# octree-nn/octfusion

Measured on AMD Instinct MI355X. Metric: denoising-steps/sec (depth-8 octree, batch 8), higher is better.
Workload: dtype f32 storage, fp16x3 products (fp16 hi + lo operand pairs = 22 significand bits, three fp16 MFMAs per product, fp32 accumulate)

## Files before the change

include/ofx.h:

```cpp
#ifndef OFX_H_
#define OFX_H_

#include <stddef.h>
#include <stdint.h>

#ifdef __cplusplus
extern "C" {
#endif

#define OFX_OK 0
#define OFX_EINVAL (-1)
#define OFX_ELAUNCH (-2)
#define OFX_ENODEV (-3)

#define OFX_ACT_NONE 0
#define OFX_ACT_SILU 1
#define OFX_ACT_GELU 2

#define OFX_MAX_DEPTH 16

int ofx_version(void);
const char* ofx_status_string(int status);
int ofx_device_check(void);
const char* ofx_build_hash(void);
// ... 72 lines not shown
int ofx_graphconv_bwd_weight(const float* x, int64_t ldx, int cin, int64_t n_nodes, const int32_t* nbr,
                             const int32_t* seg_ptr, const int32_t* col, const int32_t* nbr_ext,
                             const int32_t* multi_seg, int64_t n_multi, float* aux, const float* type_frac, int64_t ldt,
                             int nt_pad, const float* dy, int64_t ldy, int cout, float* dWp, int64_t Kp, void* ws,
                             size_t ws_bytes, void* stream);
int ofx_gn_backward(const float* x, int64_t ldx, const float* dy, int64_t ldy, int64_t n, int C,
                    const int32_t* batch_id, int batch_size, const float* count, int groups, float count_eps,
                    const float* mean, const float* rstd, const float* w, const float* bias, int act, double* sums,
                    float* coef, float* dx, int64_t lddx, float* dgamma, float* dbeta, void* stream);
int ofx_gemm_tn_f32(const float* P, int64_t ldp, const float* Q, int64_t ldq, int64_t rows, int64_t K, int64_t N,
                    float* out, void* ws, size_t ws_bytes, void* stream);
int ofx_table_reverse_count(const int32_t* nbr, int64_t n_out, int ndir, int64_t n_in, int32_t* rev_cnt, void* stream);
int ofx_table_reverse_fill(const int32_t* nbr, int64_t n_out, int ndir, int64_t n_in, const int32_t* rev_ptr,
                           int32_t* cursor, int32_t* rev_row, float* rev_w, void* stream);
int ofx_seg_primary_w(const int32_t* seg_ptr, const int32_t* col, const float* w, int64_t nseg, int32_t* nbr,
                      void* stream);
int ofx_seg_multi_flag_w(const int32_t* seg_ptr, const float* w, int64_t nseg, int32_t* flag, void* stream);
int ofx_seg_primary_ext_w(const int32_t* seg_ptr, const int32_t* col, const float* w, int64_t nseg, int64_t n_src,
                          const int32_t* rank, int32_t* nbr_ext, int32_t* multi_seg, void* stream);
int ofx_gridconv_bwd_data(const float* dy, int64_t ldy, int cout, int64_t n_out, int64_t n_in, const int32_t* nbr_rev,
                          const int32_t* rev_ptr, const int32_t* rev_row, const float* rev_w,
                          const int32_t* nbr_ext_rev, const int32_t* multi_seg, int64_t n_multi, float* aux,
                          const float* WpT, int cin, float* dx, int64_t ldx, void* ws, size_t ws_bytes, void* stream);
int ofx_gridconv_bwd_weight(const float* x, int64_t ldx, int cin, int64_t n_in, int64_t n_out, const int32_t* nbr27,
                            const int32_t* nbr27_ext, const float* zero_row, const float* dy, int64_t ldy, int cout,
                            float* dWp, void* ws, size_t ws_bytes, void* stream);
int ofx_adamw_step(float* param, const float* grad, float* exp_avg, float* exp_avg_sq, int64_t n, float lr,
                   float beta1, float beta2, float eps, float weight_decay, int step, void* stream);
int ofx_ema_update(float* ema, const float* param, int64_t n, float beta, void* stream);
typedef struct OfxAdamRow {
  float* param;
  const float* grad;
  float* exp_avg;
  float* exp_avg_sq;
  float* ema;
  int64_t n;
} OfxAdamRow;
int ofx_adamw_ema_multi(const OfxAdamRow* rows, int64_t n_rows, float lr, float beta1, float beta2, float eps,
                        float weight_decay, int step, float ema_beta, void* stream);
int ofx_adamw_ema_multi_chunk(void);
int ofx_adamw_ema_multi_rows(void);
int64_t ofx_mse_grad_partials(int64_t n);
int ofx_mse_grad(const float* y, const float* target, float* dy, double* partials, double* loss_out, int64_t n,
                 void* stream);
int ofx_mpu_eval(const ofx_tree_t* tree, int depth_start, int depth_end, const float* pts, int64_t n_pts,
                 const float* code, float* sdf, uint8_t* mask, void* stream);
int ofx_mpu_eval_grid(const ofx_tree_t* tree, int depth_start, int depth_end, const float* code, int size,
                      float step, float bbmin, int batch_index, int64_t head, int64_t count, float* sdf,
                      uint8_t* mask, void* stream);
int ofx_mpu_eval_grad(const ofx_tree_t* tree, int depth_start, int depth_end, const float* pts, int64_t n_pts,
                      const float* code, float* sdf, float* grad, uint8_t* mask, void* stream);
int ofx_mpu_backward(const ofx_tree_t* tree, int depth_start, int depth_end, const float* pts, int64_t n_pts,
                     const float* code, const float* dsdf, const float* dgrad, float* dcode, void* stream);
int ofx_octree_ce(const float* logits, int64_t ld, const int32_t* child, int64_t n, float dscale, double* sums,
                  float* dlogits, int64_t ldd, void* stream);
int ofx_sdf_reg_loss(const float* sdf, const float* grad, const float* sdf_gt, const float* grad_gt, int64_t n,
                     float w_sdf, float w_grad, double* sums, float* dsdf, float* dgrad, void* stream);
int ofx_kl_sample_fwd(const float* params, int64_t ld, const float* noise, int64_t n, int embed_dim, float* z,
                      double* kl_sum, void* stream);
int ofx_kl_sample_bwd(const float* params, int64_t ld, const float* noise, const float* dz, int64_t n,
                      int embed_dim, float kl_scale, float* dparams, int64_t ldp, void* stream);
int ofx_graph_multi_flag(const int32_t* seg_ptr, int64_t n_nodes, int32_t* flag, void* stream);
int ofx_graph_primary_ext(const int32_t* seg_ptr, const int32_t* col, int64_t n_nodes,
                          const int32_t* rank, int32_t* nbr_ext, int32_t* multi_seg, void* stream);
int ofx_graph_type_frac(const int32_t* seg_ptr, const int32_t* col, const uint8_t* node_type,
                        int64_t n_nodes, int nt, float* type_frac, int64_t ld, void* stream);

int ofx_set_precision(int mode);
int ofx_get_precision(void);
int64_t ofx_packed_floats(int64_t Kp, int64_t N);
int64_t ofx_packed_k(int64_t K);
int64_t ofx_graphconv_packed_k(int cin, int nt);
int ofx_pack_weights(const float* W, int64_t sk, int64_t sn, int64_t K, int64_t N,
                     int cin, int nt, float* Wp, int64_t Kp, void* stream);

int ofx_gemm_f32(const float* A, int64_t lda, const int32_t* a_rows, int64_t M, int64_t K,
                 const float* Wp, int64_t Kp, int64_t N, const float* bias,
                 const float* res, int64_t ldr, float* out, int64_t ldc,
                 const int32_t* out_rows, void* ws, size_t ws_bytes, void* stream);
int ofx_gemm_f32_planes(const float* A, int64_t lda, const int32_t* a_rows, int64_t M, int64_t K,
                        const float* Wp, int64_t Kp, int64_t N, const float* bias,
                        const float* res, int64_t ldr, float* out, int64_t ldc,
                        const int32_t* out_rows, void* ws, size_t ws_bytes, int out_mode, void* stream);

int ofx_graphconv_fwd(const float* x, int64_t ldx, int cin, int64_t n_nodes,
                      const int32_t* nbr, const int32_t* seg_ptr, const int32_t* col,
                      const int32_t* nbr_ext, const int32_t* multi_seg, int64_t n_multi, float* aux,
                      const float* type_frac, int64_t ldt, int nt_pad,
                      const float* Wp, int64_t Kp, int cout, const float* bias,
                      const float* emb, int64_t lde, const int32_t* batch_id,
                      const float* res, int64_t ldr, float* out, int64_t ldc,
                      double* stats , int64_t stats_ld,
                      void* ws, size_t ws_bytes, void* stream);

int ofx_graphconv_narrow_in(const float* x, int64_t ldx, int cin, int64_t n_nodes, const int32_t* seg_ptr,
                            const int32_t* col, const uint8_t* node_type, int nt, const float* W, int cout,
                            const float* bias, const int32_t* batch_id, float* out, int64_t ldc,
                            double* stats , int64_t stats_ld, void* ws, size_t ws_bytes, void* stream);
int ofx_graphconv_narrow_in_tab(const float* x, int64_t ldx, int cin, int64_t n_nodes, const int32_t* seg_ptr,
                                const int32_t* col, const int32_t* nbr_ext, const int32_t* multi_seg, int64_t n_multi,
                                void* aux, const uint8_t* node_type, int nt, const float* W, int cout, const float* bias,
                                const int32_t* batch_id, float* out, int64_t ldc, double* stats ,
                                int64_t stats_ld, void* ws, size_t ws_bytes, void* stream);
int ofx_narrow_out_pack(const float* W, int C, int nt, int cout, int pw, float* Wd, void* stream);
int ofx_narrow_out_type_term(const float* type_frac, int64_t ldt, int nt, int64_t n_nodes, const float* W, int C,
                             int cout, const float* bias, float* type_term, void* stream);
int ofx_graphconv_narrow_out(const float* P, int64_t ldp, int cout, int64_t n_nodes, const int32_t* seg_ptr,
                             const int32_t* col, const float* type_term , float* out, int64_t ldc,
                             void* stream);

int ofx_planes_split(const float* x, int64_t ldx, int64_t n, int C, int Cpad, int mode, void* out,
                     int64_t ldo_bytes, void* stream);
int ofx_planes_merge(const void* planes, int64_t ldp_bytes, int64_t n, int C, int mode, float* out, int64_t ldo,
                     void* stream);
int ofx_gn_apply_planes(const float* x, int64_t ldx, int64_t n, int C, const int32_t* batch_id, const float* mean,
                        const float* rstd, const double* sums, const float* count, int groups, float eps,
                        float count_eps, const float* w, const float* bias, int act, int mode, void* out,
                        int64_t ldo_bytes, const int32_t* seg_ptr, const int32_t* col, const int32_t* multi_seg,
                        int64_t n_multi, void* aux , const int32_t* aux_plan ,
                        int64_t aux_left, void* stream);
int ofx_gn_apply_planes_oct(const float* x, int64_t ldx, int64_t n, int C, const int32_t* batch_id, const float* mean,
                            const float* rstd, const double* sums, const float* count, int groups, float eps,
                            float count_eps, const float* w, const float* bias, int act, int mode, void* out,
                            int64_t ldo_bytes, int64_t n_multi, void* aux, const int32_t* oct_ptr,
                            const int32_t* oct_ent, int64_t n_own, int shift, const int32_t* left_head,
                            const int32_t* left_src, int64_t n_left, void* stream);
int ofx_gn_finalize_window(const double* sums, const float* count, int batch_size, int C, int groups, int c_lo,
                           int c_hi, float eps, float count_eps, float* mean, float* rstd, void* stream);
int ofx_gn_apply_planes_window(const float* x, int64_t ldx, int64_t n, int C, int c_lo, int c_hi,
                               const int32_t* batch_id, const float* mean, const float* rstd, const double* sums,
                               const float* count, int groups, float eps, float count_eps, const float* w,
                               const float* bias, int act, int mode, void* out, int64_t ldo_bytes,
                               const int32_t* seg_ptr, const int32_t* col, const int32_t* multi_seg, int64_t n_multi,
                               void* aux, const int32_t* aux_plan, int64_t aux_left, void* stream);
int ofx_gn_apply_planes_oct_window(const float* x, int64_t ldx, int64_t n, int C, int c_lo, int c_hi,
                                   const int32_t* batch_id, const float* mean, const float* rstd, const double* sums,
                                   const float* count, int groups, float eps, float count_eps, const float* w,
                                   const float* bias, int act, int mode, void* out, int64_t ldo_bytes, int64_t n_multi,
                                   void* aux, const int32_t* oct_ptr, const int32_t* oct_ent, int64_t n_own, int shift,
                                   const int32_t* left_head, const int32_t* left_src, int64_t n_left, void* stream);
int ofx_gn_apply_rows(void);
int64_t ofx_planes_packed_ktiles(int cin, int nt, int mode);
int64_t ofx_planes_packed_bytes(int cin, int nt, int cout, int mode);
int ofx_pack_weights_planes(const float* W, int64_t sk, int64_t sn, int cin, int nt, int cout, int mode, void* out,
                            void* stream);
int ofx_graphconv_fwd_planes(const void* xp, int64_t ldx_bytes, int cin, int64_t n_nodes, const int32_t* seg_ptr,
                             const int32_t* col, const int32_t* nbr_ext, const int32_t* multi_seg, int64_t n_multi,
                             void* aux, size_t aux_bytes, const void* tfp, int64_t ldt_bytes, int nt, const void* W2,
                             int cout, const float* bias, const float* emb, int64_t lde, const int32_t* batch_id,
                             const float* res, int64_t ldr, float* out, int64_t ldc, double* stats ,
                             int64_t stats_ld, void* ws, size_t ws_bytes, void* sync , size_t sync_bytes,
                             int mode, int aux_ready, void* stream);
int ofx_graphconv_fwd_planes_cus(const void* xp, int64_t ldx_bytes, int cin, int64_t n_nodes, const int32_t* seg_ptr,
                                 const int32_t* col, const int32_t* nbr_ext, const int32_t* multi_seg, int64_t n_multi,
                                 void* aux, size_t aux_bytes, const void* tfp, int64_t ldt_bytes, int nt,
                                 const void* W2, int cout, const float* bias, const float* emb, int64_t lde,
                                 const int32_t* batch_id, const float* res, int64_t ldr, float* out, int64_t ldc,
                                 double* stats , int64_t stats_ld, void* ws, size_t ws_bytes,
                                 void* sync , size_t sync_bytes, int mode, int aux_ready, int cus,
                                 void* stream);
int ofx_set_gconv_persistent(int on);
int64_t ofx_gemm_planes_packed_bytes(int K, int N, int mode);
int ofx_pack_gemm_planes(const float* W, int64_t sk, int64_t sn, int K, int N, int mode, void* out, void* stream);
int ofx_gemm_planes(const void* ap, int64_t lda_bytes, int64_t n_a, int64_t M, int K, const int32_t* row_tab,
                    const void* W2, int N, const float* bias, float* out, int64_t ldc, int out_mode, void* ws,
                    size_t ws_bytes, void* sync, size_t sync_bytes, int mode, void* stream);
int ofx_set_gconv_cus(int cus);
int ofx_gconv3_plan(int64_t n_rows, int cout, int nkt, int wm, int ni, int cus, int32_t* out, int64_t out_len);
int ofx_set_gconv2_tile(int wm);

int ofx_grid_conv_table(int mode, int depth_out, int batch_size, int32_t pad, int32_t* nbr27,
                        void* stream);
int64_t ofx_conv3d_packed_k(int cin);
int ofx_pack_conv3d(const float* W, int cin, int cout, float* Wp, void* stream);
int ofx_gridconv_fwd(const float* x, int64_t ldx, int cin, int64_t n_in, int64_t n_out,
                     const int32_t* nbr27 ,
                     const int32_t* nbr27_ext ,
                     const float* zero_row ,
                     const float* Wp, int cout, const float* bias, const float* emb, int64_t lde,
                     const int32_t* batch_id, const float* res, int64_t ldr, float* out,
                     int64_t ldc, void* ws, size_t ws_bytes, void* stream);
int ofx_gather_gemm_f32(const float* x, int64_t ldx, int cin, int ntap, int64_t n_src, int64_t n_out, const int32_t* tab,
                        const float* zero_row, const float* Wp, int64_t Kp, int cout, const float* bias,
                        const float* res, int64_t ldr, float* out, int64_t ldc, const int32_t* out_rows, void* ws,
                        size_t ws_bytes, int out_mode, void* stream);
int ofx_set_attention_split(int on);
int ofx_attention(const float* qkv, int64_t ldq, int batch_size, int T, int heads, int ch,
                  float* out, int64_t ldo, void* stream);

int ofx_attention_bwd(const float* qkv, int64_t ldq, const float* dout, int64_t ldo, int batch_size, int T, int heads,
                      int ch, float* rowstat, float* dqkv, int64_t ldd, void* stream);

int ofx_gather_mean(const float* x, int64_t ldx, int cin, int64_t n_nodes,
                    const int32_t* seg_ptr, const int32_t* col, float* col_data,
                    void* stream);

int ofx_gn_stats(const float* x, int64_t ldx, int64_t n, int C, const int32_t* batch_id,
                 int batch_size, double* sums, void* stream);
int ofx_gn_stats_acc(const float* x, int64_t ldx, int64_t n, int C, const int32_t* batch_id, int batch_size,
                     double* sums, void* stream);
int ofx_gn_finalize(const double* sums, const float* count, int batch_size, int C, int groups,
                    float eps, float count_eps, float* mean, float* rstd, void* stream);
int ofx_gn_apply(const float* x, int64_t ldx, int64_t n, int C, const int32_t* batch_id,
                 const float* mean , const float* rstd , const double* sums ,
                 const float* count, int groups, float eps, float count_eps, const float* w, const float* bias,
                 int act, float* out, int64_t ldo, void* stream);

int ofx_gn_fused_rows(const float* x, int64_t ldx, int rows_per_batch, int batch_size, int C, int groups, float eps,
                      float count_eps, const float* w, const float* bias, int act, float* out, int64_t ldo,
                      void* stream);

int ofx_set_gn_rows16(int on);

int ofx_rows_copy(const float* src, int64_t lds, const int32_t* smap, float* dst, int64_t ldd,
                  const int32_t* dmap, int64_t n, int C, void* stream);
int ofx_rows_copy_planes(const float* src, int64_t lds, const int32_t* smap, float* dst, int64_t ldd,
                         const int32_t* dmap, int64_t n, int C, int mode, void* stream);
int ofx_act(const float* x, float* y, int64_t n, int act, void* stream);
int ofx_timestep_embedding(const float* t, int batch_size, int dim, float max_period,
                           float* out, void* stream);
int ofx_learned_sinusoid(const float* t, const float* w, int batch_size, int half, float* out, void* stream);
int ofx_linear_small(const float* a, int64_t lda, int M, int K, const float* W, int64_t ldw, int N, const float* bias,
                     const float* res, int64_t ldr, int act_in, int act_out, float* out, int64_t ldo, void* stream);
int ofx_ddim_eps_update(float* x, const float* eps, const float* coef, float* x0_out, int64_t n,
                        void* stream);
int ofx_ddim_x0_update(float* x, const float* x0, const float* noise, const float* coef,
                       int64_t n, void* stream);

size_t ofx_mc_ws_bytes(int batch, int size);
int ofx_mc_count(const float* sdf, int batch, int size, float level, void* ws, int64_t* counts, void* stream);
int ofx_mc_emit(const float* sdf, int batch, int size, float level, float step, float bbmin, float scale, void* ws,
                const int64_t* vert_off, const int64_t* tri_off, float* verts, int32_t* faces, void* stream);
int ofx_mc_table_host(int8_t* tri_table, uint8_t* ntri);

size_t ofx_mesh_cc_ws_bytes(int64_t total_verts, int64_t total_faces, int batch);
int ofx_mesh_cc_label(const int32_t* faces, const int64_t* vert_off, const int64_t* tri_off, int batch,
                      int64_t total_verts, int64_t total_faces, int32_t* label, void* ws, int32_t* status,
                      void* stream);
int ofx_mesh_cc_table(const int32_t* faces, const int32_t* label, const int64_t* vert_off, const int64_t* tri_off,
                      int batch, int64_t total_verts, int64_t total_faces, int32_t* comp_of_vert, int32_t* comp_off,
                      void* ws, const int32_t* status, void* stream);
int ofx_mesh_cc_stats(const float* verts, const int32_t* faces, const int32_t* label, const int64_t* vert_off,
                      const int64_t* tri_off, int batch, int64_t total_verts, int64_t total_faces, int64_t n_comp,
                      int32_t* table, void* ws, const int32_t* status, void* stream);
int ofx_mesh_cc_select(const float* verts, const int32_t* faces, const int32_t* label, const int64_t* vert_off,
                       const int64_t* tri_off, int batch, int64_t total_verts, int64_t total_faces,
                       int32_t* winner_label, int64_t* keep_counts, void* ws, const int32_t* status, void* stream);
int ofx_mesh_cc_extract(const float* verts, const int32_t* faces, const int64_t* vert_off, const int64_t* tri_off,
                        int batch, int64_t total_verts, int64_t total_faces, const int64_t* new_vert_off,
                        const int64_t* new_tri_off, float* out_verts, int32_t* out_faces, void* ws,
                        const int32_t* status, void* stream);

size_t ofx_voxmesh_ws_bytes(int batch, int depth, int weld);
int ofx_voxmesh_mask_keys(const int64_t* keys, int64_t n, int batch0, int batch, int depth, void* ws, void* stream);
int ofx_voxmesh_mask_dense(const float* occ, int batch, int depth, float threshold, void* ws, void* stream);
int ofx_voxmesh_count(int batch, int depth, int weld, void* ws, int64_t* counts, void* stream);
int ofx_voxmesh_emit(int batch, int depth, int weld, void* ws, const int64_t* vert_off, const int64_t* tri_off,
                     float* verts, int32_t* faces, void* stream);

#define OFX_EMD_MAX_POINTS 2048
size_t ofx_surface_sample_ws_bytes(int batch, int64_t total_faces);
int ofx_surface_sample(const float* verts, const int32_t* faces, const int64_t* offs, const int64_t* ids, int batch,
                       int64_t total_faces, int n, uint64_t seed, int normalize, void* ws, float* out, void* stream);
int ofx_surface_sample_oriented(const float* verts, const int32_t* faces, const int64_t* offs, const int64_t* ids,
                                int batch, int64_t total_faces, int n, uint64_t seed, int normalize, void* ws,
                                float* out, float* normals, void* stream);
int ofx_nn_matrix(const float* a, int64_t na, int n, const float* b, int64_t nb, int m, float* d, void* stream);
int ofx_emd_matrix(const float* x, int64_t nx, const float* y, int64_t ny, int n, int m, float* e, void* stream);
// ... 40 lines not shown
```

octfusion_amd/_lib.py:

```python
import ctypes
import os

import torch

_HERE = os.path.dirname(os.path.abspath(__file__))
LIB_PATH = os.environ.get('OFX_LIB', os.path.join(_HERE, 'libofx.so'))

c_p = ctypes.c_void_p
c_i = ctypes.c_int
c_l = ctypes.c_int64
c_f = ctypes.c_float
c_d = ctypes.c_double
c_sz = ctypes.c_size_t
c_u64 = ctypes.c_uint64


class OfxTree(ctypes.Structure):
    _fields_ = [('depth', c_i), ('full_depth', c_i), ('batch_size', c_i),
                ('child_all', c_p), ('key_all', c_p), ('leafrank_all', c_p),
                ('nnum_host', c_p), ('nnum_nempty_host', c_p)]


class OfxAdamRow(ctypes.Structure):
    _fields_ = [('param', c_p), ('grad', c_p), ('exp_avg', c_p), ('exp_avg_sq', c_p), ('ema', c_p), ('n', c_l)]
# ... 3 lines not shown
    'ofx_version': (c_i, [], False),
    'ofx_status_string': (ctypes.c_char_p, [c_i], False),
    'ofx_device_check': (c_i, [], False),
    'ofx_build_hash': (ctypes.c_char_p, [], False),
    'ofx_probe_mfma_sustained': (c_i, [c_i, c_i, c_p, c_p, c_p], True),
    'ofx_scan_ws_bytes': (c_sz, [c_l], False),
    'ofx_scan_i32': (c_i, [c_p, c_p, c_l, c_p, c_p], True),
    'ofx_octree_full_layer': (c_i, [c_i, c_i, c_p, c_p, c_p], True),
    'ofx_octree_split': (c_i, [c_p, c_l, c_p, c_p, c_p, c_p], True),
    'ofx_octree_grow': (c_i, [c_p, c_p, c_l, c_p, c_p, c_p], True),
    'ofx_split_small_label0': (c_i, [c_p, c_i, c_i, c_p, c_p], True),
    'ofx_split_small_label1': (c_i, [c_p, c_i, c_i, c_p, c_p, c_p], True),
    'ofx_split_large_label0': (c_i, [c_p, c_l, c_p, c_p], True),
    'ofx_split_large_label1': (c_i, [c_p, c_l, c_p, c_p, c_p], True),
    'ofx_octree2voxel_cf': (c_i, [c_p, c_l, c_i, c_i, c_i, c_p, c_p], True),
    'ofx_voxel2octree_cf': (c_i, [c_p, c_i, c_i, c_i, c_p, c_l, c_p], True),
    'ofx_points_sort_ws_bytes': (c_sz, [c_l], False),
    'ofx_points_keys': (c_i, [c_p, c_l, c_p, c_i, c_l, c_i, c_p, c_p, c_p], True),
    'ofx_points_sort': (c_i, [c_p, c_p, c_l, c_p, c_p, c_p, c_sz, c_p], True),
    'ofx_octree_label_from_points': (c_i, [c_p, c_l, c_p, c_l, c_i, c_i, c_p, c_p], True),
    'ofx_octree_point_features': (c_i, [c_p, c_p, c_l, c_p, c_l, c_p, c_l, c_p, c_l, c_i, c_p, c_p, c_p, c_p], True),
    'ofx_tree_leafrank_ws_bytes': (c_sz, [c_l], False),
    'ofx_tree_leafrank': (c_i, [c_p, c_p, c_i, c_p, c_p, c_p], True),
    'ofx_graph_nodes': (c_i, [ctypes.POINTER(OfxTree), c_i, c_p, c_p, c_p, c_p, c_p], True),
    'ofx_graph_count': (c_i, [ctypes.POINTER(OfxTree), c_i, c_p, c_p], True),
    'ofx_graph_reverse_count': (c_i, [c_p, c_p, c_l, c_p, c_p], True),
    'ofx_graph_reverse_fill': (c_i, [c_p, c_p, c_l, c_p, c_p, c_p, c_p, c_p], True),
    'ofx_graph_primary_w': (c_i, [c_p, c_p, c_p, c_l, c_p, c_p], True),
    'ofx_graph_multi_flag_w': (c_i, [c_p, c_p, c_l, c_p, c_p], True),
    'ofx_graph_primary_ext_w': (c_i, [c_p, c_p, c_p, c_l, c_p, c_p, c_p, c_p], True),
    'ofx_graphconv_bwd_data': (c_i, [c_p, c_l, c_i, c_l, c_p, c_p, c_p, c_p, c_p, c_p, c_l, c_p, c_p, c_l, c_i, c_p,
                                     c_l, c_p, c_sz, c_p], True),
    'ofx_graphconv_bwd_weight': (c_i, [c_p, c_l, c_i, c_l, c_p, c_p, c_p, c_p, c_p, c_l, c_p, c_p, c_l, c_i, c_p, c_l,
                                       c_i, c_p, c_l, c_p, c_sz, c_p], True),
    'ofx_gn_backward': (c_i, [c_p, c_l, c_p, c_l, c_l, c_i, c_p, c_i, c_p, c_i, c_f, c_p, c_p, c_p, c_p, c_i, c_p, c_p,
                              c_p, c_l, c_p, c_p, c_p], True),
    'ofx_gemm_tn_f32': (c_i, [c_p, c_l, c_p, c_l, c_l, c_l, c_l, c_p, c_p, c_sz, c_p], True),
    'ofx_table_reverse_count': (c_i, [c_p, c_l, c_i, c_l, c_p, c_p], True),
    'ofx_table_reverse_fill': (c_i, [c_p, c_l, c_i, c_l, c_p, c_p, c_p, c_p, c_p], True),
    'ofx_seg_primary_w': (c_i, [c_p, c_p, c_p, c_l, c_p, c_p], True),
    'ofx_seg_multi_flag_w': (c_i, [c_p, c_p, c_l, c_p, c_p], True),
    'ofx_seg_primary_ext_w': (c_i, [c_p, c_p, c_p, c_l, c_l, c_p, c_p, c_p, c_p], True),
    'ofx_gridconv_bwd_data': (c_i, [c_p, c_l, c_i, c_l, c_l, c_p, c_p, c_p, c_p, c_p, c_p, c_l, c_p, c_p, c_i, c_p, c_l,
                                    c_p, c_sz, c_p], True),
    'ofx_gridconv_bwd_weight': (c_i, [c_p, c_l, c_i, c_l, c_l, c_p, c_p, c_p, c_p, c_l, c_i, c_p, c_p, c_sz, c_p], True),
    'ofx_attention_bwd': (c_i, [c_p, c_l, c_p, c_l, c_i, c_i, c_i, c_i, c_p, c_p, c_l, c_p], True),
    'ofx_adamw_step': (c_i, [c_p, c_p, c_p, c_p, c_l, c_f, c_f, c_f, c_f, c_f, c_i, c_p], True),
    'ofx_ema_update': (c_i, [c_p, c_p, c_l, c_f, c_p], True),
    'ofx_adamw_ema_multi': (c_i, [c_p, c_l, c_f, c_f, c_f, c_f, c_f, c_i, c_f, c_p], True),
    'ofx_adamw_ema_multi_chunk': (c_i, [], False),
    'ofx_adamw_ema_multi_rows': (c_i, [], False),
    'ofx_mse_grad_partials': (c_l, [c_l], False),
    'ofx_mse_grad': (c_i, [c_p, c_p, c_p, c_p, c_p, c_l, c_p], True),
    'ofx_gn_fused_rows': (c_i, [c_p, c_l, c_i, c_i, c_i, c_i, c_f, c_f, c_p, c_p, c_i, c_p, c_l, c_p], True),
    'ofx_set_gn_rows16': (c_i, [c_i], True),
    'ofx_mpu_eval': (c_i, [ctypes.POINTER(OfxTree), c_i, c_i, c_p, c_l, c_p, c_p, c_p, c_p], True),
    'ofx_mpu_eval_grid': (c_i, [ctypes.POINTER(OfxTree), c_i, c_i, c_p, c_i, c_f, c_f, c_i, c_l, c_l, c_p, c_p, c_p], True),
    'ofx_mpu_eval_grad': (c_i, [ctypes.POINTER(OfxTree), c_i, c_i, c_p, c_l, c_p, c_p, c_p, c_p, c_p], True),
    'ofx_mpu_backward': (c_i, [ctypes.POINTER(OfxTree), c_i, c_i, c_p, c_l, c_p, c_p, c_p, c_p, c_p], True),
    'ofx_octree_ce': (c_i, [c_p, c_l, c_p, c_l, c_f, c_p, c_p, c_l, c_p], True),
    'ofx_sdf_reg_loss': (c_i, [c_p, c_p, c_p, c_p, c_l, c_f, c_f, c_p, c_p, c_p, c_p], True),
    'ofx_kl_sample_fwd': (c_i, [c_p, c_l, c_p, c_l, c_i, c_p, c_p, c_p], True),
    'ofx_kl_sample_bwd': (c_i, [c_p, c_l, c_p, c_p, c_l, c_i, c_f, c_p, c_l, c_p], True),
    'ofx_graph_fill': (c_i, [ctypes.POINTER(OfxTree), c_i, c_p, c_p, c_p], True),
    'ofx_graph_expand': (c_i, [c_p, c_l, c_p, c_p, c_p, c_p, c_p], True),
    'ofx_graph_type_frac': (c_i, [c_p, c_p, c_p, c_l, c_i, c_p, c_l, c_p], True),
    'ofx_set_precision': (c_i, [c_i], True),
    'ofx_set_range_words': (c_i, [c_p], True),
    'ofx_get_precision': (c_i, [], False),
    'ofx_gn_apply_rows': (c_i, [], False),
    'ofx_set_attention_split': (c_i, [c_i], True),
    'ofx_gather_gemm_f32': (c_i, [c_p, c_l, c_i, c_i, c_l, c_l, c_p, c_p, c_p, c_l, c_i, c_p, c_p, c_l, c_p, c_l, c_p, c_p, c_sz, c_i, c_p], True),
    'ofx_graphconv_narrow_in_tab': (c_i, [c_p, c_l, c_i, c_l, c_p, c_p, c_p, c_p, c_l, c_p, c_p, c_i, c_p, c_i, c_p, c_p, c_p, c_l, c_p, c_l,
                                          c_p, c_sz, c_p], True),
    'ofx_graphconv_narrow_in': (c_i, [c_p, c_l, c_i, c_l, c_p, c_p, c_p, c_i, c_p, c_i, c_p, c_p, c_p, c_l, c_p, c_l, c_p, c_sz, c_p], True),
    'ofx_narrow_out_pack': (c_i, [c_p, c_i, c_i, c_i, c_i, c_p, c_p], True),
    'ofx_narrow_out_type_term': (c_i, [c_p, c_l, c_i, c_l, c_p, c_i, c_i, c_p, c_p, c_p], True),
    'ofx_graphconv_narrow_out': (c_i, [c_p, c_l, c_i, c_l, c_p, c_p, c_p, c_p, c_l, c_p], True),
    'ofx_packed_floats': (c_l, [c_l, c_l], False),
    'ofx_packed_k': (c_l, [c_l], False),
    'ofx_graphconv_packed_k': (c_l, [c_i, c_i], False),
    'ofx_pack_weights': (c_i, [c_p, c_l, c_l, c_l, c_l, c_i, c_i, c_p, c_l, c_p], True),
    'ofx_gemm_f32': (c_i, [c_p, c_l, c_p, c_l, c_l, c_p, c_l, c_l, c_p, c_p, c_l, c_p, c_l, c_p, c_p, c_sz, c_p], True),
    'ofx_gemm_f32_planes': (c_i, [c_p, c_l, c_p, c_l, c_l, c_p, c_l, c_l, c_p, c_p, c_l, c_p, c_l, c_p, c_p, c_sz, c_i, c_p], True),
    'ofx_graphconv_fwd': (c_i, [c_p, c_l, c_i, c_l, c_p, c_p, c_p, c_p, c_p, c_l, c_p, c_p, c_l, c_i, c_p, c_l,
                                c_i, c_p, c_p, c_l, c_p, c_p, c_l, c_p, c_l, c_p, c_l, c_p, c_sz, c_p], True),
    'ofx_planes_split': (c_i, [c_p, c_l, c_l, c_i, c_i, c_i, c_p, c_l, c_p], True),
    'ofx_planes_merge': (c_i, [c_p, c_l, c_l, c_i, c_i, c_p, c_l, c_p], True),
    'ofx_gn_apply_planes': (c_i, [c_p, c_l, c_l, c_i, c_p, c_p, c_p, c_p, c_p, c_i, c_f, c_f, c_p, c_p, c_i, c_i, c_p,
                                  c_l, c_p, c_p, c_p, c_l, c_p, c_p, c_l, c_p], True),
    'ofx_gn_apply_planes_oct': (c_i, [c_p, c_l, c_l, c_i, c_p, c_p, c_p, c_p, c_p, c_i, c_f, c_f, c_p, c_p, c_i, c_i, c_p,
                                      c_l, c_l, c_p, c_p, c_p, c_l, c_i, c_p, c_p, c_l, c_p], True),
    'ofx_planes_packed_ktiles': (c_l, [c_i, c_i, c_i], False),
    'ofx_planes_packed_bytes': (c_l, [c_i, c_i, c_i, c_i], False),
    'ofx_pack_weights_planes': (c_i, [c_p, c_l, c_l, c_i, c_i, c_i, c_i, c_p, c_p], True),
    'ofx_graphconv_fwd_planes': (c_i, [c_p, c_l, c_i, c_l, c_p, c_p, c_p, c_p, c_l, c_p, c_sz, c_p, c_l, c_i, c_p, c_i,
                                       c_p, c_p, c_l, c_p, c_p, c_l, c_p, c_l, c_p, c_l, c_p, c_sz, c_p, c_sz, c_i, c_i,
                                       c_p], True),
    'ofx_graphconv_fwd_planes_cus': (c_i, [c_p, c_l, c_i, c_l, c_p, c_p, c_p, c_p, c_l, c_p, c_sz, c_p, c_l, c_i, c_p,
                                           c_i, c_p, c_p, c_l, c_p, c_p, c_l, c_p, c_l, c_p, c_l, c_p, c_sz, c_p, c_sz,
                                           c_i, c_i, c_i, c_p], True),
    'ofx_gn_finalize_window': (c_i, [c_p, c_p, c_i, c_i, c_i, c_i, c_i, c_f, c_f, c_p, c_p, c_p], True),
    'ofx_gn_apply_planes_window': (c_i, [c_p, c_l, c_l, c_i, c_i, c_i, c_p, c_p, c_p, c_p, c_p, c_i, c_f, c_f, c_p, c_p,
                                         c_i, c_i, c_p, c_l, c_p, c_p, c_p, c_l, c_p, c_p, c_l, c_p], True),
    'ofx_gn_apply_planes_oct_window': (c_i, [c_p, c_l, c_l, c_i, c_i, c_i, c_p, c_p, c_p, c_p, c_p, c_i, c_f, c_f, c_p,
                                             c_p, c_i, c_i, c_p, c_l, c_l, c_p, c_p, c_p, c_l, c_i, c_p, c_p, c_l, c_p],
                                       True),
    'ofx_set_gconv_persistent': (c_i, [c_i], True),
    'ofx_set_gconv_cus': (c_i, [c_i], True),
    'ofx_gemm_planes_packed_bytes': (c_l, [c_i, c_i, c_i], False),
    'ofx_pack_gemm_planes': (c_i, [c_p, c_l, c_l, c_i, c_i, c_i, c_p, c_p], True),
    'ofx_gemm_planes': (c_i, [c_p, c_l, c_l, c_l, c_i, c_p, c_p, c_i, c_p, c_p, c_l, c_i, c_p, c_sz, c_p, c_sz, c_i, c_p], False),
    'ofx_gconv3_plan': (c_i, [c_l, c_i, c_i, c_i, c_i, c_i, c_p, c_l], False),
    'ofx_set_gconv2_tile': (c_i, [c_i], True),
    'ofx_graph_multi_flag': (c_i, [c_p, c_l, c_p, c_p], True),
    'ofx_graph_primary_ext': (c_i, [c_p, c_p, c_l, c_p, c_p, c_p, c_p], True),
    'ofx_graph_primary': (c_i, [c_p, c_p, c_l, c_p, c_p], True),
    'ofx_grid_conv_table': (c_i, [c_i, c_i, c_i, c_i, c_p, c_p], True),
    'ofx_conv3d_packed_k': (c_l, [c_i], False),
    'ofx_pack_conv3d': (c_i, [c_p, c_i, c_i, c_p, c_p], True),
    'ofx_gridconv_fwd': (c_i, [c_p, c_l, c_i, c_l, c_l, c_p, c_p, c_p, c_p, c_i, c_p, c_p, c_l, c_p, c_p, c_l, c_p,
                               c_l, c_p, c_sz, c_p], True),
    'ofx_attention': (c_i, [c_p, c_l, c_i, c_i, c_i, c_i, c_p, c_l, c_p], True),
    'ofx_gather_mean': (c_i, [c_p, c_l, c_i, c_l, c_p, c_p, c_p, c_p], True),
    'ofx_gn_stats': (c_i, [c_p, c_l, c_l, c_i, c_p, c_i, c_p, c_p], True),
    'ofx_gn_stats_acc': (c_i, [c_p, c_l, c_l, c_i, c_p, c_i, c_p, c_p], True),
    'ofx_gn_finalize': (c_i, [c_p, c_p, c_i, c_i, c_i, c_f, c_f, c_p, c_p, c_p], True),
    'ofx_gn_apply': (c_i, [c_p, c_l, c_l, c_i, c_p, c_p, c_p, c_p, c_p, c_i, c_f, c_f, c_p, c_p, c_i, c_p, c_l, c_p], True),
    'ofx_rows_copy': (c_i, [c_p, c_l, c_p, c_p, c_l, c_p, c_l, c_i, c_p], True),
    'ofx_rows_copy_planes': (c_i, [c_p, c_l, c_p, c_p, c_l, c_p, c_l, c_i, c_i, c_p], True),
    'ofx_act': (c_i, [c_p, c_p, c_l, c_i, c_p], True),
    'ofx_timestep_embedding': (c_i, [c_p, c_i, c_i, c_f, c_p, c_p], True),
    'ofx_learned_sinusoid': (c_i, [c_p, c_p, c_i, c_i, c_p, c_p], True),
    'ofx_linear_small': (c_i, [c_p, c_l, c_i, c_i, c_p, c_l, c_i, c_p, c_p, c_l, c_i, c_i, c_p, c_l, c_p], True),
    'ofx_ddim_eps_update': (c_i, [c_p, c_p, c_p, c_p, c_l, c_p], True),
    'ofx_ddim_x0_update': (c_i, [c_p, c_p, c_p, c_p, c_l, c_p], True),
    'ofx_mc_ws_bytes': (c_sz, [c_i, c_i], False),
    'ofx_mc_count': (c_i, [c_p, c_i, c_i, c_f, c_p, c_p, c_p], True),
    'ofx_mc_emit': (c_i, [c_p, c_i, c_i, c_f, c_f, c_f, c_f, c_p, c_p, c_p, c_p, c_p, c_p], True),
    'ofx_mc_table_host': (c_i, [c_p, c_p], True),
    'ofx_mesh_cc_ws_bytes': (c_sz, [c_l, c_l, c_i], False),
    'ofx_mesh_cc_label': (c_i, [c_p, c_p, c_p, c_i, c_l, c_l, c_p, c_p, c_p, c_p], True),
    'ofx_mesh_cc_table': (c_i, [c_p, c_p, c_p, c_p, c_i, c_l, c_l, c_p, c_p, c_p, c_p, c_p], True),
    'ofx_mesh_cc_stats': (c_i, [c_p, c_p, c_p, c_p, c_p, c_i, c_l, c_l, c_l, c_p, c_p, c_p, c_p], True),
    'ofx_mesh_cc_select': (c_i, [c_p, c_p, c_p, c_p, c_p, c_i, c_l, c_l, c_p, c_p, c_p, c_p, c_p], True),
    'ofx_mesh_cc_extract': (c_i, [c_p, c_p, c_p, c_p, c_i, c_l, c_l, c_p, c_p, c_p, c_p, c_p, c_p, c_p], True),
    'ofx_voxmesh_ws_bytes': (c_sz, [c_i, c_i, c_i], False),
    'ofx_voxmesh_mask_keys': (c_i, [c_p, c_l, c_i, c_i, c_i, c_p, c_p], True),
    'ofx_voxmesh_mask_dense': (c_i, [c_p, c_i, c_i, c_f, c_p, c_p], True),
    'ofx_voxmesh_count': (c_i, [c_i, c_i, c_i, c_p, c_p, c_p], True),
    'ofx_voxmesh_emit': (c_i, [c_i, c_i, c_i, c_p, c_p, c_p, c_p, c_p, c_p], True),
    'ofx_surface_sample_ws_bytes':(c_sz, [c_i, c_l], False),
    'ofx_surface_sample': (c_i, [c_p, c_p, c_p, c_p, c_i, c_l, c_i, c_u64, c_i, c_p, c_p, c_p], True),
    'ofx_surface_sample_oriented': (c_i, [c_p, c_p, c_p, c_p, c_i, c_l, c_i, c_u64, c_i, c_p, c_p, c_p, c_p], True),
    'ofx_nn_matrix': (c_i, [c_p, c_l, c_i, c_p, c_l, c_i, c_p, c_p], True),
    'ofx_emd_matrix': (c_i, [c_p, c_l, c_p, c_l, c_i, c_i, c_p, c_p], True),
    'ofx_metrics_hash': (c_u64, [c_u64, c_l, c_l, c_i], False),
    'ofx_nn_search_qpass': (c_i, [], False),
    'ofx_nn_search_tile': (c_i, [], False),
    'ofx_nn_search_splits': (c_i, [c_i, c_l, c_l], False),
    'ofx_nn_search_ws_bytes': (c_sz, [c_l], False),
    'ofx_nn_search': (c_i, [c_p, c_p, c_p, c_p, c_i, c_l, c_l, c_l, c_i, c_p, c_p, c_p, c_p], True),
    'ofx_sdf_sample_ws_bytes': (c_sz, [c_l, c_i], False),
    'ofx_sdf_sample_nodes': (c_i, [c_p, c_i, c_p, c_l, c_p, c_i, c_i, c_i, c_u64, c_l, c_p, c_f, c_p, c_p, c_p, c_p, c_p,
                                   c_p], True),
    'ofx_sdf_sample_occu': (c_i, [c_p, c_i, c_l, c_u64, c_l, c_p, c_f, c_p, c_p, c_p], True),
# ... 106 lines not shown
```

octfusion_amd/csrc/ofx_gemm.hip:

```cpp
#include "ofx_gemm_common.h"

constexpr int BM = 128;
constexpr int BK = 32;
constexpr int A_LD = BK + 4;
constexpr int MODE_DENSE = 0;
constexpr int MODE_GATHER = 1;

struct TileCoords { int split, tm, tn; };
__device__ __forceinline__ TileCoords tile_coords(const GemmArgs& g) {
  const int ntile = g.ntm * g.ntn;
  int bid = ofx_xcd_swizzle(blockIdx.x, ntile * g.nsplit);
  const int split = bid / ntile;
  bid -= split * ntile;
  const int tm = bid / g.ntn;
  return {split, tm, bid - tm * g.ntn};
}

__device__ __forceinline__ void load_a_dense(const GemmArgs& g, int64_t m0, int64_t k0, float4 (&va)[4]) {
  const int c4 = threadIdx.x & 7, r0 = threadIdx.x >> 3;
  const int64_t k = k0 + c4 * 4;
  const bool vec = ((g.lda & 3) == 0) && (k + 3 < g.K) && ((((uintptr_t)g.A) & 15) == 0);
#pragma unroll
  for (int i = 0; i < 4; ++i) {
    const int64_t m = m0 + r0 + 32 * i;
    float4 v = f4zero();
    if (m < g.M) {
      const int64_t ar = g.a_rows ? (int64_t)g.a_rows[m] : m;
      const float* p = g.A + ar * g.lda + k;
      if (vec) {
        v = *reinterpret_cast<const float4*>(p);
      } else {
        if (k + 0 < g.K) v.x = p[0];
        if (k + 1 < g.K) v.y = p[1];
        if (k + 2 < g.K) v.z = p[2];
        if (k + 3 < g.K) v.w = p[3];
      }
    }
    va[i] = v;
  }
}

template <int BN>
__device__ __forceinline__ void load_b_tile(const GemmArgs& g, int64_t n0, int64_t k0, float4 (&vb)[BN / 32]) {
#pragma unroll
  for (int i = 0; i < BN / 32; ++i) {
    const int idx = threadIdx.x + 256 * i;
    const int kql = idx / BN, n = idx % BN;
    const int64_t nn = n0 + n;
    vb[i] = (nn < g.N) ? *reinterpret_cast<const float4*>(g.Wp + (((k0 >> 2) + kql) * g.N + nn) * 4) : f4zero();
  }
}

template <int WM, int WN, int MI, int NI>
__global__ void __launch_bounds__(256, 2) gemm_dense_generic_kernel(const GemmArgs g) {
  constexpr int BN = WN * NI * 32;
  static_assert(WM * MI * 32 == BM, "BM");
  extern __shared__ __attribute__((aligned(16))) float smem[];
  float* As = smem;
  float* Bs = smem + 2 * BM * A_LD;

  const TileCoords tc = tile_coords(g);
  const int split = tc.split;
  const int64_t m0 = (int64_t)tc.tm * BM, n0 = (int64_t)tc.tn * BN;

  const int lane = threadIdx.x & 63, wid = threadIdx.x >> 6;
  const int wm = wid / WN, wn = wid % WN;
  const int l31 = lane & 31, h = lane >> 5;
  const int c4 = threadIdx.x & 7, r0 = threadIdx.x >> 3;

  f32x16 acc[MI][NI];
#pragma unroll
  for (int i = 0; i < MI; ++i)
#pragma unroll
    for (int j = 0; j < NI; ++j)
#pragma unroll
      for (int r = 0; r < 16; ++r) acc[i][j][r] = 0.f;

  float4 va[4];
  float4 vb[BN / 32];
  const int nkt_all = (int)(g.Kp / BK);
  const int kt_begin = split * g.kt_per_split;
  const int kt_end = (kt_begin + g.kt_per_split < nkt_all) ? kt_begin + g.kt_per_split : nkt_all;

// ... 205 lines not shown
        va2 = ldg4(xp + src_off(ia2, ldx, n_src, aux_delta) + cc);
        va3 = ldg4(xp + src_off(ia3, ldx, n_src, aux_delta) + cc);
      }
      const int ktw0 = MODE == MODE_DENSE ? g_begin : d0 * tpd + g_begin / ndir;
      load_w(wp + (int64_t)ktw0 * 8 * Ncols * 4);
    }
    stage(a_st, b_st);
    ia0 = ib0; ia1 = ib1; ia2 = ib2; ia3 = ib3;
    __syncthreads();

    for (int kt = g_begin; kt < g_end; ++kt) {
      const int buf = (kt - g_begin) & 1;
      const int ktn = kt + 1 < nkt_g ? kt + 1 : nkt_g - 1;
      const int dn = ktn % ndir;
      const int d2 = (kt + 2 < nkt_g ? kt + 2 : nkt_g - 1) % ndir;
      if (MODE == MODE_DENSE) {
        int cc = ktn * BK + c4 * 4;
        cc = cc < kclamp ? cc : kclamp;
        va0 = ldg4(dp0 + cc); va1 = ldg4(dp1 + cc); va2 = ldg4(dp2 + cc); va3 = ldg4(dp3 + cc);
      } else {
        ib0 = t0[d2]; ib1 = t1[d2]; ib2 = t2[d2]; ib3 = t3[d2];
        const int cc = (ktn / ndir) * BK + c4 * 4;
        va0 = ldg4(xp + src_off(ia0, ldx, n_src, aux_delta) + cc);
        va1 = ldg4(xp + src_off(ia1, ldx, n_src, aux_delta) + cc);
        va2 = ldg4(xp + src_off(ia2, ldx, n_src, aux_delta) + cc);
        va3 = ldg4(xp + src_off(ia3, ldx, n_src, aux_delta) + cc);
      }
      const int ktw = MODE == MODE_DENSE ? ktn : dn * tpd + ktn / ndir;
      load_w(wp + (int64_t)ktw * 8 * Ncols * 4);
      __builtin_amdgcn_sched_barrier(0);
      mfma_tile<WM, WN, MI, NI>(a_ld + buf * BM * A_LD, b_ld + buf * 8 * BN * 4, acc);
      __builtin_amdgcn_sched_barrier(0);
      stage(a_st + (buf ^ 1) * BM * A_LD, b_st + (buf ^ 1) * 8 * BN * 4);
      ia0 = ib0; ia1 = ib1; ia2 = ib2; ia3 = ib3;
      __syncthreads();
    }
  }

  for (int kt = t_begin; kt < kt_end; ++kt) {
    const int cc = (kt - nkt_g) * BK + c4 * 4;
    va0 = ldg4(tfp + m_0 * ldt + cc);
    va1 = ldg4(tfp + m_1 * ldt + cc);
    va2 = ldg4(tfp + m_2 * ldt + cc);
    va3 = ldg4(tfp + m_3 * ldt + cc);
    load_w(wp + (int64_t)kt * 8 * Ncols * 4);
    stage(a_st, b_st);
    __syncthreads();
    mfma_tile<WM, WN, MI, NI>(a_ld, b_ld, acc);
    __syncthreads();
  }

  epilogue_store<WM, WN, MI, NI>(g, acc, m0, n0, wm, wn, l31, h, split);
}


typedef __bf16 bf16x8_t __attribute__((ext_vector_type(8)));
typedef _Float16 f16x8h_t __attribute__((ext_vector_type(8)));
typedef unsigned u32x4h __attribute__((ext_vector_type(4)));

template <int H16>
__device__ __forceinline__ void split16x4(const float4& v, uint2& hi, uint2& lo) {
  if constexpr (H16 == 0) {
    hi.x = g2_pk_bf16(v.x, v.y);
    hi.y = g2_pk_bf16(v.z, v.w);
    const float hx = g2_bf16_lo(hi.x), hy = g2_bf16_hi(hi.x);
    const float hz = g2_bf16_lo(hi.y), hw = g2_bf16_hi(hi.y);
    lo.x = g2_pk_bf16(v.x - hx, v.y - hy);
    lo.y = g2_pk_bf16(v.z - hz, v.w - hw);
  } else {
    hi.x = g2_pk_f16(v.x, v.y);
    hi.y = g2_pk_f16(v.z, v.w);
    lo.x = g2_pk_f16(v.x - g2_f16_lo(hi.x), v.y - g2_f16_hi(hi.x));
    lo.y = g2_pk_f16(v.z - g2_f16_lo(hi.y), v.w - g2_f16_hi(hi.y));
  }
}
template <int H16>
__device__ __forceinline__ f32x16 mfma16(u32x4h a, u32x4h b, f32x16 c) {
  if constexpr (H16 == 0)
    return __builtin_amdgcn_mfma_f32_32x32x16_bf16(__builtin_bit_cast(bf16x8_t, a), __builtin_bit_cast(bf16x8_t, b), c, 0, 0, 0);
  else
    return __builtin_amdgcn_mfma_f32_32x32x16_f16(__builtin_bit_cast(f16x8h_t, a), __builtin_bit_cast(f16x8h_t, b), c, 0, 0, 0);
}

template <int MODE, int WM, int WN, int MI, int NI, int H16>
__global__ void __launch_bounds__(256, 2) gemm_pairs_x3_kernel(const GemmArgs g) {
  constexpr int BN = WN * NI * 32;
  constexpr int A_BYTES = BM * 80;
  constexpr int BUF_BYTES = 2 * A_BYTES;
  static_assert(WM * MI * 32 == BM, "BM");
  extern __shared__ __attribute__((aligned(16))) char smem8[];
  typedef unsigned u32x4 __attribute__((ext_vector_type(4)));
  typedef const u32x4 __attribute__((address_space(1)))* gqp;

  const TileCoords tc = tile_coords(g);
  const int split = tc.split;
  const int64_t m0 = (int64_t)tc.tm * BM, n0 = (int64_t)tc.tn * BN;

  const int lane = threadIdx.x & 63, wid = threadIdx.x >> 6;
  const int wm = wid / WN, wn = wid % WN;
  const int l31 = lane & 31, h = lane >> 5;
  const int c4 = threadIdx.x & 7;
  const int r0 = ((threadIdx.x >> 4) & 3) + 8 * (threadIdx.x >> 6) + 4 * ((threadIdx.x >> 3) & 1);

  const gfp xp = (gfp)sgpr64((uint64_t)(MODE == MODE_DENSE ? g.A : g.x));
  const gfp tfp = (gfp)sgpr64((uint64_t)g.tf);
  const gqp w16 = (gqp)sgpr64((uint64_t)g.W16);
  const gip tab = (gip)sgpr64((uint64_t)g.nbr_ext);
  const int64_t ldx = (int64_t)sgpr64((uint64_t)(MODE == MODE_DENSE ? g.lda : g.ldx));
  const int64_t ldt = (int64_t)sgpr64((uint64_t)g.ldt), n_src = (int64_t)sgpr64((uint64_t)g.n_src);
  const int64_t Ncols = (int64_t)sgpr64((uint64_t)g.N);
  const int64_t lo_off = (int64_t)sgpr64((uint64_t)(g.Kp / 8 * g.N));
  const int64_t aux_delta = (int64_t)sgpr64((uint64_t)((g.aux - g.x) - g.n_src * g.ldx));
  const int ndir = g.ndir;

  f32x16 acc[MI][NI];
#pragma unroll
  for (int i = 0; i < MI; ++i)
#pragma unroll
    for (int j = 0; j < NI; ++j)
#pragma unroll
      for (int r = 0; r < 16; ++r) acc[i][j][r] = 0.f;

  const int nkt_all = (int)(g.Kp / BK);
  const int kt_begin = split * g.kt_per_split;
  const int kt_end = (kt_begin + g.kt_per_split < nkt_all) ? kt_begin + g.kt_per_split : nkt_all;
  const int tpd = MODE == MODE_DENSE ? nkt_all : g.cin / BK;
  const int nkt_g = MODE == MODE_DENSE ? nkt_all : ndir * tpd;
  const int g_begin = kt_begin < nkt_g ? kt_begin : nkt_g;
  const int g_end = kt_end < nkt_g ? kt_end : nkt_g;
  const int t_begin = kt_begin > nkt_g ? kt_begin : nkt_g;

  int64_t m_0 = m0 + r0, m_1 = m_0 + 32, m_2 = m_0 + 64, m_3 = m_0 + 96;
  const int64_t mmax = g.M - 1;
  m_0 = m_0 < mmax ? m_0 : mmax; m_1 = m_1 < mmax ? m_1 : mmax;
  m_2 = m_2 < mmax ? m_2 : mmax; m_3 = m_3 < mmax ? m_3 : mmax;
  const gip t0 = tab + m_0 * ndir;
  const gip t1 = tab + m_1 * ndir;
  const gip t2 = tab + m_2 * ndir;
  const gip t3 = tab + m_3 * ndir;
  int64_t dr0 = m_0, dr1 = m_1, dr2 = m_2, dr3 = m_3;
  if (MODE == MODE_DENSE && g.a_rows) { dr0 = g.a_rows[m_0]; dr1 = g.a_rows[m_1]; dr2 = g.a_rows[m_2]; dr3 = g.a_rows[m_3]; }
  const gfp dp0 = xp + dr0 * ldx, dp1 = xp + dr1 * ldx, dp2 = xp + dr2 * ldx, dp3 = xp + dr3 * ldx;
  const int kclamp = (int)g.K - 4;

  int64_t bcol[NI];
#pragma unroll
  for (int j = 0; j < NI; ++j) {
    int64_t nn = n0 + (wn * NI + j) * 32 + l31;
    bcol[j] = (nn < Ncols ? nn : Ncols - 1) + (int64_t)h * Ncols;
  }
  char* const a_st = smem8 + (r0 * 80 + c4 * 8);
  const char* const a_ld = smem8 + ((wm * MI * 32 + l31) * 80 + 16 * h);

  struct BFrag { u32x4 h[2][NI], l[2][NI]; };
  struct RegSet { float4 a0, a1, a2, a3; };
  struct IdxSet { uint32_t i0, i1, i2, i3; };

  auto load_bfrag = [&](int ktw, BFrag& F) {
    const gqp wk = w16 + (int64_t)ktw * 4 * Ncols;
#pragma unroll
    for (int c = 0; c < 2; ++c)
#pragma unroll
      for (int j = 0; j < NI; ++j) {
        F.h[c][j] = wk[(int64_t)(2 * c) * Ncols + bcol[j]];
        F.l[c][j] = wk[lo_off + (int64_t)(2 * c) * Ncols + bcol[j]];
      }
  };
  auto store_a = [&](int buf, const RegSet& R) {
    char* a = a_st + buf * BUF_BYTES;
    uint2 hi, lo;
    split16x4<H16>(R.a0, hi, lo);
    *reinterpret_cast<uint2*>(a) = hi; *reinterpret_cast<uint2*>(a + A_BYTES) = lo;
    split16x4<H16>(R.a1, hi, lo);
    *reinterpret_cast<uint2*>(a + 32 * 80) = hi; *reinterpret_cast<uint2*>(a + 32 * 80 + A_BYTES) = lo;
    split16x4<H16>(R.a2, hi, lo);
    *reinterpret_cast<uint2*>(a + 64 * 80) = hi; *reinterpret_cast<uint2*>(a + 64 * 80 + A_BYTES) = lo;
    split16x4<H16>(R.a3, hi, lo);
    *reinterpret_cast<uint2*>(a + 96 * 80) = hi; *reinterpret_cast<uint2*>(a + 96 * 80 + A_BYTES) = lo;
  };
  auto compute = [&](int buf, const BFrag& F) {
    const char* a = a_ld + buf * BUF_BYTES;
    u32x4h ah[2][MI], al[2][MI];
#pragma unroll
    for (int c = 0; c < 2; ++c)
#pragma unroll
      for (int i = 0; i < MI; ++i) {
        ah[c][i] = *reinterpret_cast<const u32x4h*>(a + i * 32 * 80 + 32 * c);
        al[c][i] = *reinterpret_cast<const u32x4h*>(a + i * 32 * 80 + 32 * c + A_BYTES);
      }
#pragma unroll
    for (int c = 0; c < 2; ++c) {
#pragma unroll
      for (int i = 0; i < MI; ++i)
#pragma unroll
        for (int j = 0; j < NI; ++j)
          acc[i][j] = mfma16<H16>(al[c][i], F.h[c][j], acc[i][j]);
#pragma unroll
      for (int i = 0; i < MI; ++i)
#pragma unroll
        for (int j = 0; j < NI; ++j)
          acc[i][j] = mfma16<H16>(ah[c][i], F.l[c][j], acc[i][j]);
#pragma unroll
      for (int i = 0; i < MI; ++i)
#pragma unroll
        for (int j = 0; j < NI; ++j)
          acc[i][j] = mfma16<H16>(ah[c][i], F.h[c][j], acc[i][j]);
    }
  };

  if (g_begin < g_end) {
    RegSet R0, R1;
    IdxSet I0 = {0, 0, 0, 0}, I1 = {0, 0, 0, 0};
    BFrag F0, F1;
    auto clampg = [&](int it) { return it < nkt_g ? it : nkt_g - 1; };
    auto ktw_of = [&](int it) {
      const int itc = clampg(it);
      return MODE == MODE_DENSE ? itc : (itc % ndir) * tpd + itc / ndir;
    };
    auto load_idx = [&](int it, IdxSet& I) {
      if (MODE == MODE_DENSE) return;
      const int dc = clampg(it) % ndir;
      I.i0 = (uint32_t)t0[dc]; I.i1 = (uint32_t)t1[dc]; I.i2 = (uint32_t)t2[dc]; I.i3 = (uint32_t)t3[dc];
    };
    auto load_rows = [&](int it, const IdxSet& I, RegSet& R) {
      const int itc = clampg(it);
      if (MODE == MODE_DENSE) {
        int cc = itc * BK + c4 * 4;
        cc = cc < kclamp ? cc : kclamp;
        R.a0 = ldg4(dp0 + cc); R.a1 = ldg4(dp1 + cc); R.a2 = ldg4(dp2 + cc); R.a3 = ldg4(dp3 + cc);
      } else {
        const int cc = (itc / ndir) * BK + c4 * 4;
        R.a0 = ldg4(xp + src_off(I.i0, ldx, n_src, aux_delta) + cc);
        R.a1 = ldg4(xp + src_off(I.i1, ldx, n_src, aux_delta) + cc);
        R.a2 = ldg4(xp + src_off(I.i2, ldx, n_src, aux_delta) + cc);
        R.a3 = ldg4(xp + src_off(I.i3, ldx, n_src, aux_delta) + cc);
      }
    };
    auto load_bchunk = [&](int ktw, int c, BFrag& F) {
      const gqp wk = w16 + (int64_t)ktw * 4 * Ncols + (int64_t)(2 * c) * Ncols;
#pragma unroll
      for (int j = 0; j < NI; ++j) { F.h[c][j] = wk[bcol[j]]; F.l[c][j] = wk[lo_off + bcol[j]]; }
    };
    auto store_half = [&](int buf, const float4& v0, const float4& v1, int row_off) {
      char* a = a_st + buf * BUF_BYTES + row_off * 80;
      uint2 hi, lo;
      split16x4<H16>(v0, hi, lo);
      *reinterpret_cast<uint2*>(a) = hi; *reinterpret_cast<uint2*>(a + A_BYTES) = lo;
      split16x4<H16>(v1, hi, lo);
      *reinterpret_cast<uint2*>(a + 32 * 80) = hi; *reinterpret_cast<uint2*>(a + 32 * 80 + A_BYTES) = lo;
    };
#define OFX_FENCE() __builtin_amdgcn_sched_barrier(0)
    auto step = [&](int it, int buf, const IdxSet& Iuse, IdxSet& Iload, const BFrag& Fcur, BFrag& Fnext,
                    RegSet& Rnew, const RegSet& Rold) {
      const char* a = a_ld + buf * BUF_BYTES;
      const int ktw = ktw_of(it + 1);
      u32x4h ah[2][MI], al[2][MI];
#pragma unroll
      for (int c = 0; c < 2; ++c)
#pragma unroll
        for (int i = 0; i < MI; ++i) {
          ah[c][i] = *reinterpret_cast<const u32x4h*>(a + i * 32 * 80 + 32 * c);
          al[c][i] = *reinterpret_cast<const u32x4h*>(a + i * 32 * 80 + 32 * c + A_BYTES);
        }
      load_idx(it + 3, Iload);
      OFX_FENCE();
#define OFX_MFMA_GROUP(AOP, BOP, C)                                                                        \
      _Pragma("unroll") for (int i = 0; i < MI; ++i)                                                        \
        _Pragma("unroll") for (int j = 0; j < NI; ++j)                                                      \
          acc[i][j] = mfma16<H16>(AOP[C][i], Fcur.BOP[C][j], acc[i][j]);
      OFX_MFMA_GROUP(al, h, 0);
      OFX_FENCE();
      load_bchunk(ktw, 0, Fnext);
      OFX_FENCE();
      OFX_MFMA_GROUP(ah, l, 0);
      OFX_FENCE();
      load_bchunk(ktw, 1, Fnext);
      OFX_FENCE();
      OFX_MFMA_GROUP(ah, h, 0);
      OFX_FENCE();
      load_rows(it + 2, Iuse, Rnew);
      OFX_FENCE();
      OFX_MFMA_GROUP(al, h, 1);
      OFX_FENCE();
      store_half(buf ^ 1, Rold.a0, Rold.a1, 0);
      OFX_FENCE();
      OFX_MFMA_GROUP(ah, l, 1);
      OFX_FENCE();
      store_half(buf ^ 1, Rold.a2, Rold.a3, 64);
      OFX_FENCE();
      OFX_MFMA_GROUP(ah, h, 1);
#undef OFX_MFMA_GROUP
      __syncthreads();
    };

    load_idx(g_begin, I0);
    load_idx(g_begin + 1, I1);
    OFX_FENCE();
    load_rows(g_begin, I0, R0);
    load_bchunk(ktw_of(g_begin), 0, F0);
    load_bchunk(ktw_of(g_begin), 1, F0);
    OFX_FENCE();
    load_idx(g_begin + 2, I0);
    OFX_FENCE();
    load_rows(g_begin + 1, I1, R1);
    OFX_FENCE();
    store_half(0, R0.a0, R0.a1, 0);
    store_half(0, R0.a2, R0.a3, 64);
    __syncthreads();
    int it = g_begin;
    for (; it + 1 < g_end; it += 2) {
      step(it, 0, I0, I1, F0, F1, R0, R1);
      step(it + 1, 1, I1, I0, F1, F0, R1, R0);
    }
    if (it < g_end) step(it, 0, I0, I1, F0, F1, R0, R1);
    __syncthreads();
#undef OFX_FENCE
  }

  for (int kt = t_begin; kt < kt_end; ++kt) {
    const int cc = (kt - nkt_g) * BK + c4 * 4;
    RegSet R;
    BFrag F;
    R.a0 = ldg4(tfp + m_0 * ldt + cc);
    R.a1 = ldg4(tfp + m_1 * ldt + cc);
    R.a2 = ldg4(tfp + m_2 * ldt + cc);
    R.a3 = ldg4(tfp + m_3 * ldt + cc);
    load_bfrag(kt, F);
    store_a(0, R);
    __syncthreads();
    compute(0, F);
    __syncthreads();
  }

  epilogue_store<WM, WN, MI, NI>(g, acc, m0, n0, wm, wn, l31, h, split);
}

__device__ __forceinline__ uint32_t bf16_rne_bits(float f) {
  const uint32_t u = __float_as_uint(f);
  return (u + 0x7fffu + ((u >> 16) & 1u)) >> 16;
}
__global__ void pack_bf16x3_kernel(const float* __restrict__ Wp, int64_t Kp, int64_t N, uint16_t* __restrict__ W16,
                                   int h16) {
  const int64_t total = Kp * N;
  const float wscale = h16 ? reinterpret_cast<const float*>(W16 + 2 * total)[1] : 1.f;
  for (int64_t t = (int64_t)blockIdx.x * blockDim.x + threadIdx.x; t < total; t += (int64_t)gridDim.x * blockDim.x) {
    const int64_t kg = t / (N * 8), rem = t - kg * N * 8;
    const int64_t n = rem / 8;
    const int kk = (int)(rem - n * 8);
    const int64_t k = kg * 8 + kk;
    const float w = Wp[((k >> 2) * N + n) * 4 + (k & 3)];
    if (h16) {
      const float ws = g2_sat16(w * wscale);
      const _Float16 hi = (_Float16)ws;
      const _Float16 lo = (_Float16)(ws - (float)hi);
      W16[t] = __builtin_bit_cast(unsigned short, hi);
      W16[total + t] = __builtin_bit_cast(unsigned short, lo);
    } else {
      const uint32_t hi = bf16_rne_bits(w);
      const float wl = w - __uint_as_float(hi << 16);
      W16[t] = (uint16_t)hi;
      W16[total + t] = (uint16_t)bf16_rne_bits(wl);
    }
  }
}
static int g_precision = 3;
static int pack_bf16x3(const float* Wp, int64_t Kp, int64_t N, hipStream_t st) {
  uint16_t* W16 = reinterpret_cast<uint16_t*>(const_cast<float*>(Wp) + Kp * N);
  if (ofx_launch_weight_scale(Wp, 1, 0, Kp * N, 1, g_precision == 3 ? 1 : 0, const_cast<float*>(Wp) + 2 * Kp * N, st))
    return OFX_ELAUNCH;
  pack_bf16x3_kernel<<<ofx_grid(Kp * N, 256), 256, 0, st>>>(Wp, Kp, N, W16, g_precision == 3 ? 1 : 0);
  return hipGetLastError() == hipSuccess ? OFX_OK : OFX_ELAUNCH;
}

extern "C" int ofx_set_precision(int mode) {
  if (mode < 0 || mode > 3) return OFX_EINVAL;
  g_precision = mode;
  return OFX_OK;
}
extern "C" int ofx_get_precision(void) { return g_precision; }
extern "C" int64_t ofx_packed_floats(int64_t Kp, int64_t N) { return 2 * Kp * N + 32; }

__global__ void __launch_bounds__(256) multi_mean_kernel(const float* __restrict__ x, int64_t ldx, int cin,
                                                         const int32_t* __restrict__ seg_ptr,
                                                         const int32_t* __restrict__ col,
                                                         const int32_t* __restrict__ multi_seg, int64_t V,
                                                         float* __restrict__ aux, int64_t ldaux,
                                                         const float* __restrict__ w) {
  const int c4n = cin >> 2;
  const int64_t total = (V + 1) * c4n;
  for (int64_t t = (int64_t)blockIdx.x * blockDim.x + threadIdx.x; t < total; t += (int64_t)gridDim.x * blockDim.x) {
    const int64_t v = t / c4n;
    const int c = (int)(t - v * c4n) * 4;
    float4 acc = f4zero();
    if (v > 0) {
      const int64_t s = multi_seg[v - 1];
      const int32_t a = seg_ptr[s], e = seg_ptr[s + 1];
      if (w) {
        for (int32_t p = a; p < e; ++p) {
          const float wp = w[p];
          const float4 xv = *reinterpret_cast<const float4*>(x + (int64_t)col[p] * ldx + c);
          acc.x += wp * xv.x; acc.y += wp * xv.y; acc.z += wp * xv.z; acc.w += wp * xv.w;
        }
      } else {
        for (int32_t p = a; p < e; ++p) f4add(acc, *reinterpret_cast<const float4*>(x + (int64_t)col[p] * ldx + c));
        const float inv = 1.f / (float)(e - a);
        acc.x *= inv; acc.y *= inv; acc.z *= inv; acc.w *= inv;
      }
    }
    *reinterpret_cast<float4*>(aux + v * ldaux + c) = acc;
  }
}

__global__ void __launch_bounds__(256) splitk_reduce_kernel(const GemmArgs g) {
  const int64_t total = g.M * g.N;
  for (int64_t t = (int64_t)blockIdx.x * blockDim.x + threadIdx.x; t < total; t += (int64_t)gridDim.x * blockDim.x) {
    const int64_t m = t / g.N, n = t - m * g.N;
    float v = 0.f;
    for (int s = 0; s < g.nsplit; ++s) v += g.ws[(int64_t)s * total + t];
    if (g.oscale_p) v *= *g.oscale_p;
    if (g.bias) v += g.bias[n];
    if (g.emb) v += g.emb[(int64_t)g.bid[m] * g.lde + n];
    if (g.res) v += g.res[m * g.ldr + n];
    int64_t om = m;
    if (g.out_rows) { om = g.out_rows[m]; if (om < 0) continue; }
    g.out[om * g.ldc + n] = v;
  }
}

__global__ void __launch_bounds__(256) splitk_reduce_v4_kernel(const GemmArgs g) {
  const int64_t n4 = g.N >> 2, total4 = g.M * n4, total = g.M * g.N;
  for (int64_t t = (int64_t)blockIdx.x * blockDim.x + threadIdx.x; t < total4; t += (int64_t)gridDim.x * blockDim.x) {
    const int64_t m = t / n4, n = (t - m * n4) * 4;
    const float* p = g.ws + m * g.N + n;
    float4 v = f4zero();
    int s = 0;
    for (; s + 7 < g.nsplit; s += 8) {
      float4 a[8];
#pragma unroll
      for (int u = 0; u < 8; ++u) a[u] = *reinterpret_cast<const float4*>(p + (int64_t)(s + u) * total);
#pragma unroll
      for (int u = 0; u < 8; ++u) f4add(v, a[u]);
    }
    for (; s + 3 < g.nsplit; s += 4) {
      const float4 a0 = *reinterpret_cast<const float4*>(p + (int64_t)s * total);
      const float4 a1 = *reinterpret_cast<const float4*>(p + (int64_t)(s + 1) * total);
      const float4 a2 = *reinterpret_cast<const float4*>(p + (int64_t)(s + 2) * total);
      const float4 a3 = *reinterpret_cast<const float4*>(p + (int64_t)(s + 3) * total);
      f4add(v, a0); f4add(v, a1); f4add(v, a2); f4add(v, a3);
    }
    for (; s < g.nsplit; ++s) f4add(v, *reinterpret_cast<const float4*>(p + (int64_t)s * total));
    if (g.oscale_p) { const float osc = *g.oscale_p; v.x *= osc; v.y *= osc; v.z *= osc; v.w *= osc; }
    if (g.bias) f4add(v, *reinterpret_cast<const float4*>(g.bias + n));
    if (g.emb) f4add(v, *reinterpret_cast<const float4*>(g.emb + (int64_t)g.bid[m] * g.lde + n));
    if (g.res) f4add(v, *reinterpret_cast<const float4*>(g.res + m * g.ldr + n));
    int64_t om = m;
    if (g.out_rows) { om = g.out_rows[m]; if (om < 0) continue; }
    if (g.out_planes) ofx_store_planes4(g.out, om * g.ldc + n, v, g.out_planes);
    else *reinterpret_cast<float4*>(g.out + om * g.ldc + n) = v;
  }
}

template <void (*KERNEL)(const GemmArgs), size_t LDS>
static int launch_tiled(GemmArgs& g, hipStream_t st) {
  static bool attr_set[OFX_MAX_DEVICES] = {};
  if (LDS > 64 * 1024 &&
      !ofx_raise_lds_limit(reinterpret_cast<const void*>(KERNEL), (int)LDS, attr_set))
    return OFX_ELAUNCH;
  KERNEL<<<g.ntm * g.ntn * g.nsplit, 256, LDS, st>>>(g);
  return OFX_OK;
}
template <int MODE, int WM, int WN, int MI, int NI>
static int launch_cfg(GemmArgs& g, int flavour, hipStream_t st) {
  constexpr size_t lds_f32 = (2 * BM * A_LD + 2 * 8 * (WN * NI * 32) * 4) * sizeof(float);
  constexpr size_t lds_16 = 2 * (2 * BM * 80);
  switch (flavour) {
    case 3: return launch_tiled<gemm_pairs_x3_kernel<MODE, WM, WN, MI, NI, 1>, lds_16>(g, st);
    case 2: return launch_tiled<gemm_pairs_x3_kernel<MODE, WM, WN, MI, NI, 0>, lds_16>(g, st);
    case 1: return launch_tiled<gemm_fast_kernel<MODE, WM, WN, MI, NI>, lds_f32>(g, st);
  }
  if constexpr (MODE == MODE_DENSE) return launch_tiled<gemm_dense_generic_kernel<WM, WN, MI, NI>, lds_f32>(g, st);
  return OFX_EINVAL;
}

__global__ void __launch_bounds__(256) stats_reduce_kernel(const float* __restrict__ part, int64_t nwr, int wr_rows,
                                                            int64_t N, const int32_t* __restrict__ bid,
                                                            double* __restrict__ stats, int64_t stats_ld) {
  __shared__ double red[3][64][2];
  const int c = threadIdx.x & 63, rg = threadIdx.x >> 6;
  const int64_t n = (int64_t)blockIdx.y * 64 + c;
  const int64_t w0 = (int64_t)blockIdx.x * 64;
  const int64_t nc = n < N ? n : N - 1;
  int b[16];
  float2 v[16];
#pragma unroll
  for (int i = 0; i < 16; ++i) {
    const int64_t w = w0 + rg * 16 + i;
    const int64_t wc = w < nwr ? w : nwr - 1;
    b[i] = bid[wc * wr_rows];
    v[i] = *reinterpret_cast<const float2*>(part + (wc * N + nc) * 2);
    if (w >= nwr) { b[i] = -1; v[i] = make_float2(0.f, 0.f); }
  }
  const int bfirst = bid[w0 * wr_rows];
  bool ok = true;
#pragma unroll
  for (int i = 0; i < 16; ++i) ok = ok && (b[i] == bfirst || b[i] < 0);
  const bool uni = __syncthreads_and(ok);
  auto flush = [&](int bb, double s, double q) {
    double* o = stats + ((int64_t)bb * stats_ld + n) * 2;
    unsafeAtomicAdd(o, s); unsafeAtomicAdd(o + 1, q);
  };
  if (uni) {
    double s = 0.0, q = 0.0;
#pragma unroll
    for (int i = 0; i < 16; ++i) { s += (double)v[i].x; q += (double)v[i].y; }
    if (rg > 0) { red[rg - 1][c][0] = s; red[rg - 1][c][1] = q; }
    __syncthreads();
    if (rg == 0 && n < N) {
#pragma unroll
      for (int r = 0; r < 3; ++r) { s += red[r][c][0]; q += red[r][c][1]; }
      flush(bfirst, s, q);
    }
  } else if (n < N) {
    double s = 0.0, q = 0.0;
    int sb = -1;
#pragma unroll
    for (int i = 0; i < 16; ++i) {
      if (b[i] < 0) continue;
      if (b[i] != sb) {
        if (sb >= 0) flush(sb, s, q);
        sb = b[i]; s = 0.0; q = 0.0;
      }
      s += (double)v[i].x; q += (double)v[i].y;
    }
    if (sb >= 0) flush(sb, s, q);
  }
}

int ofx_launch_stats_reduce(const GemmArgs& g, int wr_rows, hipStream_t st) {
  const int64_t nwr = ofx_cdiv(g.M, wr_rows);
  stats_reduce_kernel<<<dim3((unsigned)ofx_cdiv(nwr, 64), (unsigned)ofx_cdiv(g.N, 64)), 256, 0, st>>>(
      g.stats_part, nwr, wr_rows, g.N, g.bid, g.stats, g.stats_ld);
  OFX_LAUNCH_CHECK();
  return OFX_OK;
}

template <int MODE>
static int launch_gemm(GemmArgs& g, float* ws, size_t ws_bytes, hipStream_t st) {
  if (g.M <= 0 || g.N <= 0) return OFX_OK;
  if (MODE == MODE_GATHER && !(g.fast && g.nbr_ext && g.aux && (!g.out_rows || g.gather_out_rows))) return OFX_EINVAL;
  {
    auto al16 = [](const void* p) { return (reinterpret_cast<uintptr_t>(p) & 15) == 0; };
    g.vec4 = g.N % 4 == 0 && al16(g.out) && g.ldc % 4 == 0 && (!g.res || (al16(g.res) && g.ldr % 4 == 0)) &&
             (!g.emb || (al16(g.emb) && g.lde % 4 == 0)) && (!g.bias || al16(g.bias));
  }
  const int bn = g.N <= 32 ? 32 : (g.N <= 64 ? 64 : 128);
  g.ntm = (int)ofx_cdiv(g.M, BM);
  g.ntn = (int)ofx_cdiv(g.N, bn);
  const int nkt = (int)(g.Kp / BK);
  int nsplit = 1;
  const int tiles = g.ntm * g.ntn;
  if (ws && tiles < 256 && nkt >= 8) {
    nsplit = (int)ofx_cdiv(512, tiles);
    if (nsplit > nkt / 4) nsplit = nkt / 4;
    if (nsplit > 64) nsplit = 64;
    const size_t per = (size_t)g.M * g.N * sizeof(float);
    if ((size_t)nsplit * per > ws_bytes) nsplit = (int)(ws_bytes / per);
    if (nsplit < 2) nsplit = 1;
  }
  g.kt_per_split = (int)ofx_cdiv(nkt, nsplit);
  nsplit = (int)ofx_cdiv(nkt, g.kt_per_split);
  g.nsplit = nsplit;
  g.ws = ws;
  bool fast = true;
  if (MODE == MODE_DENSE) {
    fast = ((g.lda & 3) == 0) && ((g.K & 3) == 0) && g.K >= 4 && ((((uintptr_t)g.A) & 15) == 0);
    if (fast) { g.ndir = 1; g.n_src = 0; g.aux = g.A; g.tf = g.A; g.ldt = g.lda; g.nbr_ext = (const int32_t*)g.A; }
  }
  g.W16 = (g_precision != 1) ? reinterpret_cast<const uint16_t*>(g.Wp + g.Kp * g.N) : nullptr;
  const int wr_rows = bn == 32 ? 32 : 64;
  const int64_t nwr = ofx_cdiv(g.M, wr_rows);
  if (!(g.stats && g.vec4 && nsplit == 1 && g.stats_part &&
        (size_t)nwr * g.N * 2 * sizeof(float) <= g.stats_part_bytes && (((uintptr_t)g.stats_part) & 15) == 0))
    g.stats_part = nullptr;
  g.oscale_p = (fast && g.W16) ? g.Wp + 2 * g.Kp * g.N : nullptr;
  const int flavour = !fast ? 0 : (!g.W16 ? 1 : (g_precision == 3 ? 3 : 2));
  int rc;
  if (bn == 32) rc = launch_cfg<MODE, 4, 1, 1, 1>(g, flavour, st);
  else if (bn == 64) rc = launch_cfg<MODE, 2, 2, 2, 1>(g, flavour, st);
  else rc = launch_cfg<MODE, 2, 2, 2, 2>(g, flavour, st);
  if (rc) return rc;
  if (nsplit > 1) {
    const bool ws16 = (((uintptr_t)g.ws) & 15) == 0;
    if (g.vec4 && ws16) splitk_reduce_v4_kernel<<<ofx_grid(g.M * (g.N >> 2), 256), 256, 0, st>>>(g);
    else splitk_reduce_kernel<<<ofx_grid(g.M * g.N, 256), 256, 0, st>>>(g);
  }
  if (g.stats_part) {
    rc = ofx_launch_stats_reduce(g, wr_rows, st);
    if (rc) return rc;
  }
  OFX_LAUNCH_CHECK();
  return OFX_OK;
}

static inline int64_t pad32(int64_t v) { return (v + 31) / 32 * 32; }

extern "C" int64_t ofx_packed_k(int64_t K) { return pad32(K); }
extern "C" int64_t ofx_graphconv_packed_k(int cin, int nt) {
  return pad32(7 * (int64_t)cin) + (nt > 1 ? pad32(7 * (int64_t)nt) : 0);
}

__global__ void pack_weights_kernel(const float* __restrict__ W, int64_t sk, int64_t sn, int64_t K, int64_t N, int cin,
                                    int nt, float* __restrict__ Wp, int64_t Kp) {
  const int64_t total = (Kp / 4) * N;
  const int ntc = nt > 1 ? nt : 0;
  const int64_t Kf = (7 * (int64_t)cin + 31) / 32 * 32;
  for (int64_t t = (int64_t)blockIdx.x * blockDim.x + threadIdx.x; t < total; t += (int64_t)gridDim.x * blockDim.x) {
    const int64_t kq = t / N, n = t - kq * N;
    float v[4];
#pragma unroll
    for (int kk = 0; kk < 4; ++kk) {
      const int64_t k = kq * 4 + kk;
      int64_t src = -1;
      if (cin > 0) {
        if (k < 7 * (int64_t)cin) {
          const int64_t dir = k / cin, c = k - dir * cin;
          src = dir * (cin + ntc) + c;
        } else if (k >= Kf && ntc > 0 && k - Kf < 7 * (int64_t)ntc) {
          const int64_t kt = k - Kf, dir = kt / ntc, ty = kt - dir * ntc;
          src = dir * (cin + ntc) + cin + ty;
        }
      } else if (k < K) {
        src = k;
      }
      v[kk] = src >= 0 ? W[src * sk + n * sn] : 0.f;
    }
    *reinterpret_cast<float4*>(Wp + t * 4) = make_float4(v[0], v[1], v[2], v[3]);
  }
}

extern "C" int ofx_pack_weights(const float* W, int64_t sk, int64_t sn, int64_t K, int64_t N, int cin, int nt,
                                float* Wp, int64_t Kp, void* stream) {
  if (!W || !Wp || K < 1 || N < 1 || (Kp & 31) || cin < 0 || nt < 0) return OFX_EINVAL;
  if (cin > 0) {
    if (Kp != ofx_graphconv_packed_k(cin, nt) || K != 7 * (int64_t)(cin + (nt > 1 ? nt : 0))) return OFX_EINVAL;
  } else if (Kp != pad32(K)) {
    return OFX_EINVAL;
  }
  if (((uintptr_t)Wp & 15) != 0) return OFX_EINVAL;
  pack_weights_kernel<<<ofx_grid((Kp / 4) * N, 256), 256, 0, ofx_stream(stream)>>>(W, sk, sn, K, N, cin, nt, Wp, Kp);
  if (int rc = pack_bf16x3(Wp, Kp, N, ofx_stream(stream))) return rc;
  OFX_LAUNCH_CHECK();
  return OFX_OK;
}

__global__ void pack_conv3d_kernel(const float* __restrict__ W, int cin, int64_t N, float* __restrict__ Wp, int64_t Kp) {
  const int64_t total = (Kp / 4) * N;
  for (int64_t t = (int64_t)blockIdx.x * blockDim.x + threadIdx.x; t < total; t += (int64_t)gridDim.x * blockDim.x) {
    const int64_t kq = t / N, n = t - kq * N;
    float v[4];
#pragma unroll
    for (int kk = 0; kk < 4; ++kk) {
      const int64_t k = kq * 4 + kk;
      float w = 0.f;
      if (k < 27 * (int64_t)cin) {
        const int64_t tap = k / cin, c = k - tap * cin;
        w = W[(n * cin + c) * 27 + tap];
      }
      v[kk] = w;
    }
    *reinterpret_cast<float4*>(Wp + t * 4) = make_float4(v[0], v[1], v[2], v[3]);
  }
}

extern "C" int64_t ofx_conv3d_packed_k(int cin) { return pad32(27 * (int64_t)cin); }

extern "C" int ofx_pack_conv3d(const float* W, int cin, int cout, float* Wp, void* stream) {
  if (!W || !Wp || cin < 1 || cout < 1 || ((uintptr_t)Wp & 15)) return OFX_EINVAL;
  const int64_t Kp = ofx_conv3d_packed_k(cin);
  pack_conv3d_kernel<<<ofx_grid((Kp / 4) * cout, 256), 256, 0, ofx_stream(stream)>>>(W, cin, cout, Wp, Kp);
  if (int rc = pack_bf16x3(Wp, Kp, cout, ofx_stream(stream))) return rc;
  OFX_LAUNCH_CHECK();
  return OFX_OK;
}

extern "C" int ofx_gemm_f32_planes(const float* A, int64_t lda, const int32_t* a_rows, int64_t M, int64_t K,
                                   const float* Wp, int64_t Kp, int64_t N, const float* bias, const float* res, int64_t ldr,
                                   float* out, int64_t ldc, const int32_t* out_rows, void* ws, size_t ws_bytes,
                                   int out_mode, void* stream) {
  if (M == 0 && K >= 1 && N >= 1) return OFX_OK;
  if (M < 0 || K < 1 || N < 1 || !Wp || !out || (M > 0 && !A) || Kp != pad32(K) || lda < K || ldc < N ||
      (res && ldr < N) || ((uintptr_t)Wp & 15))
    return OFX_EINVAL;
  if (out_mode != 0 && out_mode != 2 && out_mode != 3) return OFX_EINVAL;
  if (out_mode && ((N & 3) || (ldc & 31) || ((uintptr_t)out & 127) || (res && ((ldr & 3) || ((uintptr_t)res & 15))) ||
                   (bias && ((uintptr_t)bias & 15)) || ((uintptr_t)ws & 15)))
    return OFX_EINVAL;
  GemmArgs g = {};
  g.A = A; g.lda = lda; g.a_rows = a_rows;
  g.M = M; g.K = K; g.Wp = Wp; g.Kp = Kp; g.N = N; g.bias = bias;
  g.res = res; g.ldr = ldr; g.out = out; g.ldc = ldc; g.out_rows = out_rows; g.out_planes = out_mode;
  return launch_gemm<MODE_DENSE>(g, (float*)ws, ws_bytes, ofx_stream(stream));
}
extern "C" int ofx_gemm_f32(const float* A, int64_t lda, const int32_t* a_rows, int64_t M, int64_t K, const float* Wp,
                            int64_t Kp, int64_t N, const float* bias, const float* res, int64_t ldr, float* out,
                            int64_t ldc, const int32_t* out_rows, void* ws, size_t ws_bytes, void* stream) {
  return ofx_gemm_f32_planes(A, lda, a_rows, M, K, Wp, Kp, N, bias, res, ldr, out, ldc, out_rows, ws, ws_bytes, 0, stream);
}

static int gather_common(GemmArgs& g, const float* x, int64_t ldx, int cin, int ndir, int64_t n_rows,
                         const int32_t* nbr, const int32_t* seg_ptr, const int32_t* col, const float* Wp, int64_t Kp,
                         int cout, const float* bias, const float* emb, int64_t lde, const int32_t* batch_id,
                         const float* res, int64_t ldr, float* out, int64_t ldc) {
  if (n_rows < 0 || cin < 1 || cout < 1 || !x || !nbr || !Wp || !out || ldx < cin || ldc < cout ||
      (res && ldr < cout) || (emb && (!batch_id || lde < cout)) || ((uintptr_t)Wp & 15))
    return OFX_EINVAL;
  g.x = x; g.ldx = ldx; g.cin = cin; g.ndir = ndir;
  g.fast = (cin % 32 == 0) && ((ldx & 3) == 0) && (((uintptr_t)x & 15) == 0);
  g.nbr = nbr; g.seg_ptr = seg_ptr; g.col = col;
  g.Kf = pad32((int64_t)ndir * cin);
  g.M = n_rows; g.K = Kp; g.Wp = Wp; g.Kp = Kp; g.N = cout; g.bias = bias;
  g.emb = emb; g.lde = lde; g.bid = batch_id; g.res = res; g.ldr = ldr; g.out = out; g.ldc = ldc;
  return OFX_OK;
}

__device__ __forceinline__ float gather_elem(const GemmArgs& g, int64_t row, int64_t k) {
  if (k >= (int64_t)g.ndir * g.cin) return 0.f;
  const int dir = (int)(k / g.cin), c = (int)(k - (int64_t)dir * g.cin);
  const int32_t nb = g.nbr[row * g.ndir + dir];
  if (nb >= 0) return g.x[(int64_t)nb * g.ldx + c];
  if (nb == -1) return 0.f;
  const int64_t s = row * g.ndir + dir;
  const int32_t a = g.seg_ptr[s], e = g.seg_ptr[s + 1];
  float acc = 0.f;
  if (g.edge_w) {
    for (int32_t p = a; p < e; ++p) acc += g.edge_w[p] * g.x[(int64_t)g.col[p] * g.ldx + c];
    return acc;
  }
  for (int32_t p = a; p < e; ++p) acc += g.x[(int64_t)g.col[p] * g.ldx + c];
  if (e - a > 1) acc /= (float)(e - a);
  return acc;
}
__global__ void __launch_bounds__(256) col_rows_kernel(const GemmArgs g, int64_t row0, int64_t rows,
                                                       float* __restrict__ colbuf) {
  const int64_t k4n = g.Kp >> 2, total = rows * k4n;
  for (int64_t t = (int64_t)blockIdx.x * blockDim.x + threadIdx.x; t < total; t += (int64_t)gridDim.x * blockDim.x) {
    const int64_t r = t / k4n, k = (t - r * k4n) * 4;
    const int64_t row = row0 + r;
    float v[4];
#pragma unroll
    for (int kk = 0; kk < 4; ++kk)
      v[kk] = (k + kk < g.Kf) ? gather_elem(g, row, k + kk) : g.tf[row * g.ldt + (k + kk - g.Kf)];
    *reinterpret_cast<float4*>(colbuf + t * 4) = make_float4(v[0], v[1], v[2], v[3]);
  }
}

static int launch_gather_via_col(const GemmArgs& g, float* ws, size_t ws_bytes, hipStream_t st) {
  if (!ws || (((uintptr_t)ws) & 15)) return OFX_EINVAL;
  size_t tail = ws_bytes / 8;
  if (tail > (size_t(16) << 20)) tail = size_t(16) << 20;
  tail &= ~size_t(15);
  const size_t row_bytes = (size_t)g.Kp * sizeof(float);
  int64_t chunk = (int64_t)((ws_bytes - tail) / row_bytes) / 128 * 128;
  if (chunk < 128) return OFX_EINVAL;
  float* tail_ws = reinterpret_cast<float*>(reinterpret_cast<char*>(ws) + (ws_bytes - tail));
  for (int64_t r0 = 0; r0 < g.M; r0 += chunk) {
    const int64_t rows = g.M - r0 < chunk ? g.M - r0 : chunk;
    col_rows_kernel<<<ofx_grid(rows * (g.Kp >> 2), 256), 256, 0, st>>>(g, r0, rows, ws);
    GemmArgs d = {};
    d.A = ws; d.lda = g.Kp; d.M = rows; d.K = g.Kp; d.Wp = g.Wp; d.Kp = g.Kp; d.N = g.N; d.bias = g.bias;
    d.emb = g.emb; d.lde = g.lde; d.bid = g.bid ? g.bid + r0 : nullptr;
    d.res = g.res ? g.res + r0 * g.ldr : nullptr; d.ldr = g.ldr;
    d.out = g.out + r0 * g.ldc; d.ldc = g.ldc;
    d.stats = g.stats; d.stats_ld = g.stats_ld;
    if (g.stats) { d.stats_part = tail_ws; d.stats_part_bytes = tail; }
    const int rc = launch_gemm<MODE_DENSE>(d, g.stats ? nullptr : tail_ws, tail, st);
    if (rc) return rc;
  }
  return OFX_OK;
}

extern "C" int ofx_graphconv_fwd(const float* x, int64_t ldx, int cin, int64_t n_nodes, const int32_t* nbr,
                                 const int32_t* seg_ptr, const int32_t* col, const int32_t* nbr_ext,
                                 const int32_t* multi_seg, int64_t n_multi, float* aux, const float* type_frac,
                                 int64_t ldt, int nt_pad, const float* Wp, int64_t Kp, int cout, const float* bias,
// ... 358 lines not shown
    a.rows_per_slice = ofx_cdiv(ofx_cdiv(rows, slices), 32) * 32;
    const int sl = (int)ofx_cdiv(rows, a.rows_per_slice);
    launch_tn<true>(a, dim3((unsigned)ofx_cdiv(Kp, 128), (unsigned)ofx_cdiv(cout, 128), (unsigned)sl), st);
    tn_reduce_kernel<<<ofx_grid(total, 256), 256, 0, st>>>(a.part, sl, total, dWp, first ? 0 : 1);
    first = 0;
  }
  OFX_LAUNCH_CHECK();
  return OFX_OK;
}

extern "C" int ofx_gemm_tn_f32(const float* P, int64_t ldp, const float* Q, int64_t ldq, int64_t rows, int64_t K,
                               int64_t N, float* out, void* ws, size_t ws_bytes, void* stream) {
  if (rows < 0 || K < 4 || N < 4 || (K & 3) || (N & 3) || !out || !ws || ldp < K || ldq < N || ((ldp | ldq) & 3) ||
      (rows > 0 && (!P || !Q)) || (((uintptr_t)P | (uintptr_t)Q | (uintptr_t)ws) & 15))
    return OFX_EINVAL;
  hipStream_t st = ofx_stream(stream);
  const int64_t total = K * N;
  if (rows == 0) {
    if (hipMemsetAsync(out, 0, (size_t)total * sizeof(float), st) != hipSuccess) return OFX_ELAUNCH;
    return OFX_OK;
  }
  const int tiles = (int)(ofx_cdiv(K, 128) * ofx_cdiv(N, 128));
  int slices = (int)ofx_cdiv(1024, tiles);
  if (slices > 256) slices = 256;
  if (slices > (int)ofx_cdiv(rows, 32)) slices = (int)ofx_cdiv(rows, 32);
  while (slices > 1 && (size_t)slices * total * sizeof(float) > ws_bytes) --slices;
  if ((size_t)slices * total * sizeof(float) > ws_bytes) return OFX_EINVAL;
  TnArgs a = {};
  a.P = P; a.ldp = ldp; a.Q = Q; a.ldq = ldq; a.Kp = K; a.N = N; a.Kf = K; a.rows = rows; a.row0 = 0;
  a.rows_per_slice = ofx_cdiv(ofx_cdiv(rows, slices), 32) * 32;
  slices = (int)ofx_cdiv(rows, a.rows_per_slice);
  a.part = (float*)ws;
  launch_tn<true>(a, dim3((unsigned)ofx_cdiv(K, 128), (unsigned)ofx_cdiv(N, 128), (unsigned)slices), st);
  tn_reduce_kernel<<<ofx_grid(total, 256), 256, 0, st>>>(a.part, slices, total, out, 0);
  OFX_LAUNCH_CHECK();
  return OFX_OK;
}

extern "C" int ofx_gridconv_fwd(const float* x, int64_t ldx, int cin, int64_t n_in, int64_t n_out,
                                const int32_t* nbr27, const int32_t* nbr27_ext, const float* zero_row,
                                const float* Wp, int cout,
                                const float* bias, const float* emb, int64_t lde, const int32_t* batch_id,
                                const float* res, int64_t ldr, float* out, int64_t ldc, void* ws, size_t ws_bytes,
                                void* stream) {
  if (n_out == 0 && cin >= 1 && cout >= 1) return OFX_OK;
  GemmArgs g = {};
  const int64_t Kp = ofx_conv3d_packed_k(cin);
  int rc = gather_common(g, x, ldx, cin, 27, n_out, nbr27 ? nbr27 : nbr27_ext, nullptr, nullptr, Wp, Kp, cout, bias,
                         emb, lde, batch_id, res, ldr, out, ldc);
  if (rc) return rc;
  if (n_in < 1) return OFX_EINVAL;
  if (g.fast && nbr27_ext && zero_row && (((uintptr_t)zero_row & 15) == 0)) {
    g.nbr_ext = nbr27_ext; g.aux = zero_row; g.ldaux = ldx; g.n_src = n_in;
    g.tf = x; g.ldt = ldx;
    return launch_gemm<MODE_GATHER>(g, (float*)ws, ws_bytes, ofx_stream(stream));
  }
  if (!nbr27) return OFX_EINVAL;
  return launch_gather_via_col(g, (float*)ws, ws_bytes, ofx_stream(stream));
}

extern "C" int ofx_gather_gemm_f32(const float* x, int64_t ldx, int cin, int ntap, int64_t n_src, int64_t n_out,
                                   const int32_t* tab, const float* zero_row, const float* Wp, int64_t Kp, int cout,
                                   const float* bias, const float* res, int64_t ldr, float* out, int64_t ldc,
                                   const int32_t* out_rows, void* ws, size_t ws_bytes, int out_mode, void* stream) {
  if (n_out == 0 && cin >= 1 && cout >= 1) return OFX_OK;
  if (ntap < 1 || ntap > 64 || n_src < 1 || !tab || !zero_row || ((uintptr_t)zero_row & 15) || (cin & 31) || (ldx & 3) ||
      ((uintptr_t)x & 15) || Kp != pad32((int64_t)ntap * cin))
    return OFX_EINVAL;
  if (out_mode != 0 && out_mode != 2 && out_mode != 3) return OFX_EINVAL;
  if (out_mode && ((cout & 3) || (ldc & 31) || ((uintptr_t)out & 127) || (res && ((ldr & 3) || ((uintptr_t)res & 15))) ||
                   (bias && ((uintptr_t)bias & 15)) || ((uintptr_t)ws & 15)))
    return OFX_EINVAL;
  GemmArgs g = {};
  int rc = gather_common(g, x, ldx, cin, ntap, n_out, tab, nullptr, nullptr, Wp, Kp, cout, bias, nullptr, 0, nullptr, res,
                         ldr, out, ldc);
  if (rc) return rc;
  if (!g.fast) return OFX_EINVAL;
  g.nbr_ext = tab; g.aux = zero_row; g.ldaux = ldx; g.n_src = n_src;
  g.tf = x; g.ldt = ldx;
  g.out_rows = out_rows; g.gather_out_rows = 1; g.out_planes = out_mode;
  return launch_gemm<MODE_GATHER>(g, (float*)ws, ws_bytes, ofx_stream(stream));
}

__global__ void __launch_bounds__(256) gather_mean_kernel(const float* __restrict__ x, int64_t ldx, int cin, int64_t nseg,
                                                          const int32_t* __restrict__ seg_ptr,
                                                          const int32_t* __restrict__ col, float* __restrict__ out) {
  const int c4n = cin >> 2;
  const int64_t total = nseg * c4n;
  for (int64_t t = (int64_t)blockIdx.x * blockDim.x + threadIdx.x; t < total; t += (int64_t)gridDim.x * blockDim.x) {
    const int64_t s = t / c4n;
    const int c = (int)(t - s * c4n) * 4;
    const int32_t a = seg_ptr[s], e = seg_ptr[s + 1];
    float4 acc = f4zero();
    for (int32_t p = a; p < e; ++p) f4add(acc, *reinterpret_cast<const float4*>(x + (int64_t)col[p] * ldx + c));
    if (e - a > 1) {
      const float inv = 1.f / (float)(e - a);
      acc.x *= inv; acc.y *= inv; acc.z *= inv; acc.w *= inv;
    }
    *reinterpret_cast<float4*>(out + s * cin + c) = acc;
  }
}
__global__ void __launch_bounds__(256) gather_mean_scalar_kernel(const float* __restrict__ x, int64_t ldx, int cin,
                                                                 int64_t nseg, const int32_t* __restrict__ seg_ptr,
                                                                 const int32_t* __restrict__ col,
                                                                 float* __restrict__ out) {
  const int64_t total = nseg * cin;
  for (int64_t t = (int64_t)blockIdx.x * blockDim.x + threadIdx.x; t < total; t += (int64_t)gridDim.x * blockDim.x) {
    const int64_t s = t / cin;
    const int c = (int)(t - s * cin);
    const int32_t a = seg_ptr[s], e = seg_ptr[s + 1];
    float acc = 0.f;
    for (int32_t p = a; p < e; ++p) acc += x[(int64_t)col[p] * ldx + c];
    if (e - a > 1) acc /= (float)(e - a);
    out[t] = acc;
  }
}

extern "C" int ofx_gather_mean(const float* x, int64_t ldx, int cin, int64_t n_nodes, const int32_t* seg_ptr,
                               const int32_t* col, float* col_data, void* stream) {
  if (!x || !seg_ptr || !col || !col_data || cin < 1 || ldx < cin || n_nodes < 0) return OFX_EINVAL;
  const int64_t nseg = n_nodes * 7;
  hipStream_t st = ofx_stream(stream);
  const bool vec = (cin % 4 == 0) && ((ldx & 3) == 0) && (((uintptr_t)x & 15) == 0) && (((uintptr_t)col_data & 15) == 0);
  if (vec)
    gather_mean_kernel<<<ofx_grid(nseg * (cin / 4), 256), 256, 0, st>>>(x, ldx, cin, nseg, seg_ptr, col, col_data);
  else
    gather_mean_scalar_kernel<<<ofx_grid(nseg * cin, 256), 256, 0, st>>>(x, ldx, cin, nseg, seg_ptr, col, col_data);
  OFX_LAUNCH_CHECK();
  return OFX_OK;
}
```

octfusion_amd/csrc/ofx_gemm_common.h:

```cpp
#pragma once
#include "ofx_common.h"

typedef float f32x16 __attribute__((ext_vector_type(16)));

struct GemmArgs {
  const float* A; int64_t lda; const int32_t* a_rows;
  const float* x; int64_t ldx; int cin; int ndir; int fast;
  const int32_t* nbr;
  const int32_t* seg_ptr; const int32_t* col;
  const float* edge_w;
  const float* tf; int64_t ldt; int64_t Kf;
  const int32_t* nbr_ext;
  const float* aux; int64_t ldaux; int64_t n_src;
  int64_t M, K;
  const float* Wp; int64_t Kp, N;
  const uint16_t* W16;
  const float* oscale_p;
  const float* bias;
  const float* emb; int64_t lde; const int32_t* bid;
  const float* res; int64_t ldr;
  float* out; int64_t ldc; const int32_t* out_rows;
  int gather_out_rows;
  int out_planes;
  double* stats; int64_t stats_ld;
  int ntm, ntn, nsplit, kt_per_split;
  float* ws;
  int vec4;
  float* stats_part; size_t stats_part_bytes;
};

static __global__ void __launch_bounds__(256) weight_absmax_kernel(const float* __restrict__ W, int64_t sk, int64_t sn, int64_t K,
                                                            int64_t N, unsigned* __restrict__ acc) {
  __shared__ float red[256];
  float m = 0.f;
  for (int64_t t = (int64_t)blockIdx.x * 256 + threadIdx.x; t < K * N; t += (int64_t)gridDim.x * 256) {
    const float a = fabsf(W[(t / N) * sk + (t % N) * sn]);
    if (a <= 3.0e38f) m = fmaxf(m, a);
  }
  red[threadIdx.x] = m;
  __syncthreads();
  for (int o = 128; o > 0; o >>= 1) {
    if ((int)threadIdx.x < o) red[threadIdx.x] = fmaxf(red[threadIdx.x], red[threadIdx.x + o]);
    __syncthreads();
  }
  if (threadIdx.x == 0) atomicMax(acc, __float_as_uint(red[0]));
}
static __global__ void weight_scale_finish_kernel(int fp16_operands, float* __restrict__ scale) {
  const float mx = __uint_as_float(reinterpret_cast<const unsigned*>(scale)[0]);
  float s = 1.f;
  if (fp16_operands && mx > 0.f) {
    int e;
    frexpf(mx, &e);
    int sh = 15 - e;
    sh = sh < -60 ? -60 : (sh > 60 ? 60 : sh);
    s = ldexpf(1.f, sh);
  }
  scale[0] = 1.f / s;
  scale[1] = s;
}
static inline int ofx_launch_weight_scale(const float* W, int64_t sk, int64_t sn, int64_t K, int64_t N, int fp16_operands,
                                          float* scale, hipStream_t st) {
  if (hipMemsetAsync(scale, 0, sizeof(float), st) != hipSuccess) return OFX_ELAUNCH;
  int64_t nb = (K * N + 256 * 16 - 1) / (256 * 16);
  nb = nb < 1 ? 1 : (nb > 1024 ? 1024 : nb);
  weight_absmax_kernel<<<(unsigned)nb, 256, 0, st>>>(W, sk, sn, K, N, reinterpret_cast<unsigned*>(scale));
  if (hipGetLastError() != hipSuccess) return OFX_ELAUNCH;
  weight_scale_finish_kernel<<<1, 1, 0, st>>>(fp16_operands, scale);
  if (hipGetLastError() != hipSuccess) return OFX_ELAUNCH;
  return OFX_OK;
}


__device__ __forceinline__ unsigned g2_pk_bf16(float a, float b) {
  unsigned r;
  asm("v_cvt_pk_bf16_f32 %0, %1, %2" : "=v"(r) : "v"(a), "v"(b));
  return r;
}
__device__ __forceinline__ unsigned g2_pk_f16(float a, float b) {
  const _Float16 x = (_Float16)a, y = (_Float16)b;
  return (unsigned)__builtin_bit_cast(unsigned short, x) | ((unsigned)__builtin_bit_cast(unsigned short, y) << 16);
}
__device__ __forceinline__ float g2_bf16_lo(unsigned p) { return __uint_as_float(p << 16); }
__device__ __forceinline__ float g2_bf16_hi(unsigned p) { return __uint_as_float(p & 0xffff0000u); }
__device__ __forceinline__ float g2_f16_lo(unsigned p) { return (float)__builtin_bit_cast(_Float16, (unsigned short)(p & 0xffffu)); }
__device__ __forceinline__ float g2_f16_hi(unsigned p) { return (float)__builtin_bit_cast(_Float16, (unsigned short)(p >> 16)); }
__device__ __forceinline__ float g2_sat16(float v) { return fminf(fmaxf(v, -65504.f), 65504.f); }
__device__ __forceinline__ void g2_split2(int mode, float a, float b, unsigned& hi, unsigned& lo) {
  if (mode == 3) {
    hi = g2_pk_f16(a, b);
    lo = g2_pk_f16(a - g2_f16_lo(hi), b - g2_f16_hi(hi));
  } else {
    hi = g2_pk_bf16(a, b);
    lo = g2_pk_bf16(a - g2_bf16_lo(hi), b - g2_bf16_hi(hi));
  }
}
__device__ __forceinline__ void g2_join2(int mode, unsigned hi, unsigned lo, float& a, float& b) {
  if (mode == 3) { a = g2_f16_lo(hi) + g2_f16_lo(lo); b = g2_f16_hi(hi) + g2_f16_hi(lo); }
  else { a = g2_bf16_lo(hi) + g2_bf16_lo(lo); b = g2_bf16_hi(hi) + g2_bf16_hi(lo); }
}
__host__ __device__ static inline bool g2_pairs(int mode) { return mode == 2 || mode == 3; }

__device__ __forceinline__ void ofx_store_planes4(float* base, int64_t f, const float4& v, int mode) {
  unsigned h0, h1, l0, l1;
  g2_split2(mode, v.x, v.y, h0, l0);
  g2_split2(mode, v.z, v.w, h1, l1);
  char* o = reinterpret_cast<char*>(base) + (f >> 5) * 128 + (f & 31) * 2;
  *reinterpret_cast<uint2*>(o) = make_uint2(h0, h1);
  *reinterpret_cast<uint2*>(o + 64) = make_uint2(l0, l1);
}

__device__ __forceinline__ int ofx_xcd_swizzle(int bid, int n) {
  const int q = n / 8, r = n % 8, xcd = bid % 8, j = bid / 8;
  return (xcd < r ? xcd * (q + 1) : r * (q + 1) + (xcd - r) * q) + j;
// ... 183 lines not shown
```

octfusion_amd/csrc/ofx_norm.hip:

```cpp
#include "ofx_planes.h"

constexpr int GN_ROWS_PER_BLOCK = 64;

static inline int64_t gn_stats_rows(int64_t n, int batch_size, int C = 128) {
  const int64_t chunks = (n + GN_ROWS_PER_BLOCK - 1) / GN_ROWS_PER_BLOCK;
  const int64_t bytes_per_batch = n * (int64_t)C * 4 / (batch_size > 0 ? batch_size : 1);
  int64_t per_batch = bytes_per_batch / (512 << 10);
  per_batch = per_batch < 8 ? 8 : (per_batch > 128 ? 128 : per_batch);
  int64_t cap = per_batch * (int64_t)batch_size;
  if (cap < 64) cap = 64;
  return chunks <= cap ? GN_ROWS_PER_BLOCK : GN_ROWS_PER_BLOCK * ((chunks + cap - 1) / cap);
}

__global__ void __launch_bounds__(256) gn_stats_kernel(const float* __restrict__ x, int64_t ldx, int64_t n, int C,
                                                       const int32_t* __restrict__ bid, double* __restrict__ sums,
                                                       int64_t rpb) {
  __shared__ int sb[256];
  __shared__ float sv[256][8];
  const int CT = C >> 2;
  const int RP = 256 / CT;
  const int cl = threadIdx.x % CT, rl = threadIdx.x / CT;
  int cb = -1;
  float s[4] = {0, 0, 0, 0}, q[4] = {0, 0, 0, 0};
  auto flush_direct = [&](int b, const float* ps, const float* pq) {
    if (b < 0) return;
    double* o = sums + ((int64_t)b * C + cl * 4) * 2;
#pragma unroll
    for (int k = 0; k < 4; ++k) {
      unsafeAtomicAdd(o + 2 * k, (double)ps[k]);
      unsafeAtomicAdd(o + 2 * k + 1, (double)pq[k]);
    }
  };
  auto accum = [&](int b, const float4& v) {
    if (b != cb) {
      flush_direct(cb, s, q);
      cb = b;
      s[0] = s[1] = s[2] = s[3] = 0.f;
      q[0] = q[1] = q[2] = q[3] = 0.f;
    }
    s[0] += v.x; s[1] += v.y; s[2] += v.z; s[3] += v.w;
    q[0] += v.x * v.x; q[1] += v.y * v.y; q[2] += v.z * v.z; q[3] += v.w * v.w;
  };
  const int64_t r_begin = (int64_t)blockIdx.x * rpb;
  const int64_t r_end = r_begin + rpb < n ? r_begin + rpb : n;
  if (rl < RP) {
    int64_t r = r_begin + rl;
    for (; r + 3 * (int64_t)RP < r_end; r += 4 * (int64_t)RP) {
      const int b0 = bid[r], b1 = bid[r + RP], b2 = bid[r + 2 * RP], b3 = bid[r + 3 * RP];
      const float4 v0 = *reinterpret_cast<const float4*>(x + r * ldx + cl * 4);
      const float4 v1 = *reinterpret_cast<const float4*>(x + (r + RP) * ldx + cl * 4);
      const float4 v2 = *reinterpret_cast<const float4*>(x + (r + 2 * RP) * ldx + cl * 4);
      const float4 v3 = *reinterpret_cast<const float4*>(x + (r + 3 * RP) * ldx + cl * 4);
      accum(b0, v0); accum(b1, v1); accum(b2, v2); accum(b3, v3);
    }
    for (; r < r_end; r += RP) accum(bid[r], *reinterpret_cast<const float4*>(x + r * ldx + cl * 4));
  }
  sb[threadIdx.x] = (rl < RP) ? cb : -1;
#pragma unroll
  for (int k = 0; k < 4; ++k) { sv[threadIdx.x][k] = s[k]; sv[threadIdx.x][4 + k] = q[k]; }
  __syncthreads();
  if (rl == 0) {
    double ds[4] = {0, 0, 0, 0}, dq[4] = {0, 0, 0, 0};
    for (int j = 0; j < RP; ++j) {
      const int t = j * CT + cl;
      const int b = sb[t];
      if (b < 0) continue;
      if (b == cb) {
#pragma unroll
        for (int k = 0; k < 4; ++k) { ds[k] += (double)sv[t][k]; dq[k] += (double)sv[t][4 + k]; }
      } else {
        flush_direct(b, &sv[t][0], &sv[t][4]);
      }
    }
    if (cb >= 0) {
      double* o = sums + ((int64_t)cb * C + cl * 4) * 2;
#pragma unroll
      for (int k = 0; k < 4; ++k) { unsafeAtomicAdd(o + 2 * k, ds[k]); unsafeAtomicAdd(o + 2 * k + 1, dq[k]); }
    }
  }
}

extern "C" int ofx_gn_stats(const float* x, int64_t ldx, int64_t n, int C, const int32_t* batch_id, int batch_size,
                            double* sums, void* stream) {
  if (!x || !batch_id || !sums || n < 0 || C < 4 || (C & 3) || C > 1024 || ldx < C || (ldx & 3) ||
      ((uintptr_t)x & 15) || batch_size < 1)
    return OFX_EINVAL;
  hipStream_t st = ofx_stream(stream);
  if (hipMemsetAsync(sums, 0, sizeof(double) * 2 * (size_t)batch_size * C, st) != hipSuccess) return OFX_ELAUNCH;
  if (n > 0) gn_stats_kernel<<<(int)ofx_cdiv(n, gn_stats_rows(n, batch_size, C)), 256, 0, st>>>(x, ldx, n, C, batch_id, sums,
                                                                                             gn_stats_rows(n, batch_size, C));
  OFX_LAUNCH_CHECK();
  return OFX_OK;
}

extern "C" int ofx_gn_stats_acc(const float* x, int64_t ldx, int64_t n, int C, const int32_t* batch_id, int batch_size,
                                double* sums, void* stream) {
  if (!x || !batch_id || !sums || n < 0 || C < 4 || (C & 3) || C > 1024 || ldx < C || (ldx & 3) ||
      ((uintptr_t)x & 15) || batch_size < 1)
    return OFX_EINVAL;
  if (n > 0) gn_stats_kernel<<<(int)ofx_cdiv(n, gn_stats_rows(n, batch_size, C)), 256, 0, ofx_stream(stream)>>>(
      x, ldx, n, C, batch_id, sums, gn_stats_rows(n, batch_size, C));
  OFX_LAUNCH_CHECK();
  return OFX_OK;
}

__global__ void gn_finalize_kernel(const double* __restrict__ sums, const float* __restrict__ count, int B, int C, int G,
                                   int ld, float eps, float count_eps, float* __restrict__ mean,
                                   float* __restrict__ rstd) {
  const int cpg = C / G;
  for (int t = blockIdx.x * blockDim.x + threadIdx.x; t < B * G; t += gridDim.x * blockDim.x) {
    const int b = t / G, g = t - b * G;
    double S = 0, SS = 0;
    for (int c = g * cpg; c < (g + 1) * cpg; ++c) {
      S += sums[((int64_t)b * ld + c) * 2];
      SS += sums[((int64_t)b * ld + c) * 2 + 1];
    }
    const float cnt = count[b] * (float)cpg;
    const float inv = 1.0f / (cnt + count_eps);
    const double m = S * (double)inv;
    const double ssd = SS - 2.0 * m * S + (double)cnt * m * m;
    const double var = (ssd > 0 ? ssd : 0) * (double)inv;
    const float rs = (float)(1.0 / sqrt(var + (double)eps));
    for (int c = g * cpg; c < (g + 1) * cpg; ++c) {
      mean[(int64_t)b * ld + c] = (float)m;
      rstd[(int64_t)b * ld + c] = rs;
    }
  }
}

extern "C" int ofx_gn_finalize(const double* sums, const float* count, int batch_size, int C, int groups, float eps,
                               float count_eps, float* mean, float* rstd, void* stream) {
  if (!sums || !count || !mean || !rstd || batch_size < 1 || C < 1 || groups < 1 || C % groups) return OFX_EINVAL;
  gn_finalize_kernel<<<ofx_grid((int64_t)batch_size * groups, 64), 64, 0, ofx_stream(stream)>>>(
      sums, count, batch_size, C, groups, C, eps, count_eps, mean, rstd);
  OFX_LAUNCH_CHECK();
  return OFX_OK;
}

static bool gn_window_ok(int C, int groups, int c_lo, int c_hi, int chunk = 32) {
  if (C < 1 || groups < 1 || C % groups) return false;
  const int cpg = C / groups;
  return c_lo >= 0 && c_lo < c_hi && c_hi <= C && c_lo % chunk == 0 && c_hi % chunk == 0 && c_lo % cpg == 0 &&
         c_hi % cpg == 0;
}

extern "C" int ofx_gn_finalize_window(const double* sums, const float* count, int batch_size, int C, int groups,
                                      int c_lo, int c_hi, float eps, float count_eps, float* mean, float* rstd,
                                      void* stream) {
  if (!sums || !count || !mean || !rstd || batch_size < 1 || !gn_window_ok(C, groups, c_lo, c_hi)) return OFX_EINVAL;
  const int gw = (c_hi - c_lo) / (C / groups);
  gn_finalize_kernel<<<ofx_grid((int64_t)batch_size * gw, 64), 64, 0, ofx_stream(stream)>>>(
      sums + 2 * (int64_t)c_lo, count, batch_size, c_hi - c_lo, gw, C, eps, count_eps, mean + c_lo, rstd + c_lo);
  OFX_LAUNCH_CHECK();
  return OFX_OK;
}

__device__ __forceinline__ float ofx_apply_act(float v, int act) {
  if (act == OFX_ACT_SILU) return v / (1.f + __expf(-v));
  if (act == OFX_ACT_GELU) return 0.5f * v * (1.f + erff(v * 0.70710678118654752440f));
  return v;
}

constexpr int GN_APPLY_ROWS = 64;
struct GnFin { const double* sums; const float* count; int G; float eps, count_eps; int ld; };
__device__ __forceinline__ void gn_group_stats(const GnFin& f, int b, int g, int C, float& mean, float& rstd) {
  const int cpg = C / f.G;
  double S = 0, SS = 0;
  for (int c = g * cpg; c < (g + 1) * cpg; ++c) {
    S += f.sums[((int64_t)b * f.ld + c) * 2];
    SS += f.sums[((int64_t)b * f.ld + c) * 2 + 1];
  }
  const float cnt = f.count[b] * (float)cpg;
  const float inv = 1.0f / (cnt + f.count_eps);
  const double m = S * (double)inv;
  const double ssd = SS - 2.0 * m * S + (double)cnt * m * m;
  const double var = (ssd > 0 ? ssd : 0) * (double)inv;
  mean = (float)m;
  rstd = (float)(1.0 / sqrt(var + (double)f.eps));
}
template <int MODE, bool FIN>
__global__ void __launch_bounds__(256) gn_apply_kernel(const float* __restrict__ x, int64_t ldx, int64_t n, int C,
                                                       const int32_t* __restrict__ bid, const float* __restrict__ mean,
                                                       const float* __restrict__ rstd, const GnFin fin,
                                                       const float* __restrict__ w,
                                                       const float* __restrict__ bias, int act, char* __restrict__ out,
                                                       int64_t ldo, int64_t aux_blocks,
                                                       const int32_t* __restrict__ seg_ptr,
                                                       const int32_t* __restrict__ col,
                                                       const int32_t* __restrict__ multi_seg, int64_t n_multi,
                                                       char* __restrict__ aux, const int32_t* __restrict__ aux_plan) {
  const int CT = C >> 2, RP = 256 / CT;
  const int cl = threadIdx.x % CT, rl = threadIdx.x / CT;
  __shared__ float fin_ms[FIN ? 2 * 2 * 1024 : 1];
  constexpr int AUX_LDS = 64;
  __shared__ int aux_v[AUX_LDS], aux_n[AUX_LDS], aux_src[AUX_LDS][4];
  int fb0 = -1, fb1 = -1;
  const int64_t gT = gridDim.x;
  const int64_t a_before = aux_blocks > 0 ? ((int64_t)blockIdx.x * aux_blocks) / gT : 0;
  const bool is_aux = aux_blocks > 0 && (((int64_t)blockIdx.x + 1) * aux_blocks) / gT > a_before;
  const int64_t aux_id = a_before, main_id = (int64_t)blockIdx.x - a_before;
  const int64_t r_begin0 = main_id * GN_APPLY_ROWS;
  const int64_t r_end0 = r_begin0 + GN_APPLY_ROWS < n ? r_begin0 + GN_APPLY_ROWS : n;
  const bool pre = FIN && !is_aux && rl < RP && r_begin0 + rl + 3 * (int64_t)RP < r_end0;
  float4 pv0, pv1, pv2, pv3;
  int pb0 = 0, pb1 = 0, pb2 = 0, pb3 = 0;
  if (pre) {
    const int64_t r = r_begin0 + rl;
    const int c_ = cl * 4;
    pb0 = bid[r]; pb1 = bid[r + RP]; pb2 = bid[r + 2 * RP]; pb3 = bid[r + 3 * RP];
    pv0 = *reinterpret_cast<const float4*>(x + r * ldx + c_);
    pv1 = *reinterpret_cast<const float4*>(x + (r + RP) * ldx + c_);
    pv2 = *reinterpret_cast<const float4*>(x + (r + 2 * RP) * ldx + c_);
    pv3 = *reinterpret_cast<const float4*>(x + (r + 3 * RP) * ldx + c_);
  }
  if (FIN) {
    if (!is_aux) {
      fb0 = bid[r_begin0];
      fb1 = bid[r_end0 - 1];
    } else {
      const int64_t v0 = aux_id * RP, v1e = v0 + RP - 1 < n_multi ? v0 + RP - 1 : n_multi;
      if (n_multi > 0) {
        fb0 = bid[multi_seg[(v0 > 0 ? v0 : 1) - 1] / 7];
        fb1 = bid[multi_seg[(v1e > 0 ? v1e : 1) - 1] / 7];
      }
    }
    const int cpg = C / fin.G;
    for (int t = threadIdx.x; t < 2 * fin.G && fb0 >= 0; t += 256) {
      const int slot = t / fin.G, g = t - slot * fin.G;
      if (slot == 1 && fb1 == fb0) continue;
      float mm, rr;
      gn_group_stats(fin, slot ? fb1 : fb0, g, C, mm, rr);
      for (int cc = g * cpg; cc < (g + 1) * cpg; ++cc) {
        fin_ms[(slot * 2 + 0) * 1024 + cc] = mm;
        fin_ms[(slot * 2 + 1) * 1024 + cc] = rr;
      }
    }
    __syncthreads();
  }
  int own_b = 0, own_e = 0;
  if (!is_aux && aux && aux_plan && MODE != 0) {
    const int64_t mb_ = (n + GN_APPLY_ROWS - 1) / GN_APPLY_ROWS;
    own_b = aux_plan[main_id]; own_e = aux_plan[main_id + 1];
    const int i = own_b + (int)threadIdx.x;
    if (i < own_e && (int)threadIdx.x < AUX_LDS) {
      const int v = aux_plan[mb_ + 1 + i];
      const int64_t sgm = multi_seg[v - 1];
      const int32_t pa = seg_ptr[sgm], pz = seg_ptr[sgm + 1];
      aux_v[threadIdx.x] = v;
      aux_n[threadIdx.x] = pz - pa;
#pragma unroll
      for (int k = 0; k < 4; ++k) aux_src[threadIdx.x][k] = col[pa + k < pz ? pa + k : pa];
      if (pz - pa > 4) aux_n[threadIdx.x] = -(int)(pa + 1);
    }
  }
  const bool active = rl < RP;
  const int c = cl * 4;
  const float4 ww = *reinterpret_cast<const float4*>(w + c);
  const float4 bb = *reinterpret_cast<const float4*>(bias + c);
  int cb = -1;
  float4 m = make_float4(0.f, 0.f, 0.f, 0.f), rs = m;
  auto norm = [&](int b, const float4& v) {
    if (b != cb) {
      cb = b;
      if (FIN) {
        if (b == fb0 || b == fb1) {
          const int slot = b == fb0 ? 0 : 1;
          m = *reinterpret_cast<const float4*>(fin_ms + (slot * 2 + 0) * 1024 + c);
          rs = *reinterpret_cast<const float4*>(fin_ms + (slot * 2 + 1) * 1024 + c);
        } else {
          const int cpg = C / fin.G;
          float mm[4], rr[4];
#pragma unroll
          for (int k = 0; k < 4; ++k) {
            if (k == 0 || (c + k) / cpg != (c + k - 1) / cpg) gn_group_stats(fin, b, (c + k) / cpg, C, mm[k], rr[k]);
            else { mm[k] = mm[k - 1]; rr[k] = rr[k - 1]; }
          }
          m = make_float4(mm[0], mm[1], mm[2], mm[3]);
          rs = make_float4(rr[0], rr[1], rr[2], rr[3]);
        }
      } else {
        m = *reinterpret_cast<const float4*>(mean + (int64_t)b * fin.ld + c);
        rs = *reinterpret_cast<const float4*>(rstd + (int64_t)b * fin.ld + c);
      }
    }
    return make_float4(ofx_apply_act((v.x - m.x) * rs.x * ww.x + bb.x, act),
                       ofx_apply_act((v.y - m.y) * rs.y * ww.y + bb.y, act),
                       ofx_apply_act((v.z - m.z) * rs.z * ww.z + bb.z, act),
                       ofx_apply_act((v.w - m.w) * rs.w * ww.w + bb.w, act));
  };
  auto store = [&](char* orow, const float4& y) {
    if (MODE == 0) {
      *reinterpret_cast<float4*>(orow + (int64_t)c * 4) = y;
    } else if (MODE == 2 || MODE == 3) {
      unsigned h0, h1, l0, l1;
      g2_split2(MODE, y.x, y.y, h0, l0);
      g2_split2(MODE, y.z, y.w, h1, l1);
      char* o = orow + (c >> 5) * 128 + (c & 31) * 2;
      *reinterpret_cast<uint2*>(o) = make_uint2(h0, h1);
      *reinterpret_cast<uint2*>(o + 64) = make_uint2(l0, l1);
    } else {
      const _Float16 a0 = (_Float16)y.x, a1 = (_Float16)y.y, a2 = (_Float16)y.z, a3 = (_Float16)y.w;
      uint2 o;
      o.x = (unsigned)__builtin_bit_cast(unsigned short, a0) | ((unsigned)__builtin_bit_cast(unsigned short, a1) << 16);
      o.y = (unsigned)__builtin_bit_cast(unsigned short, a2) | ((unsigned)__builtin_bit_cast(unsigned short, a3) << 16);
      *reinterpret_cast<uint2*>(orow + c * 2) = o;
    }
  };
  auto aux_row = [&](int64_t v) {
    float4 acc = make_float4(0.f, 0.f, 0.f, 0.f);
    if (v > 0) {
      const int64_t sgm = multi_seg[v - 1];
      const int32_t pa = seg_ptr[sgm], pe = seg_ptr[sgm + 1];
      for (int32_t p0 = pa; p0 < pe; p0 += 4) {
        int64_t sr[4];
        int bb4[4];
        float4 xv[4];
#pragma unroll
        for (int k = 0; k < 4; ++k) sr[k] = col[p0 + k < pe ? p0 + k : pa];
#pragma unroll
        for (int k = 0; k < 4; ++k) {
          bb4[k] = bid[sr[k]];
          xv[k] = *reinterpret_cast<const float4*>(x + sr[k] * ldx + c);
        }
#pragma unroll
        for (int k = 0; k < 4; ++k) {
          const float4 y = norm(bb4[k], xv[k]);
          const float wgt = p0 + k < pe ? 1.f : 0.f;
          acc.x += wgt * y.x; acc.y += wgt * y.y; acc.z += wgt * y.z; acc.w += wgt * y.w;
        }
      }
      const float inv = 1.f / (float)(pe - pa);
      acc.x *= inv; acc.y *= inv; acc.z *= inv; acc.w *= inv;
    }
    store(aux + v * ldo, acc);
  };
  const int64_t mb = (n + GN_APPLY_ROWS - 1) / GN_APPLY_ROWS;
  if (is_aux) {
    if (!active) return;
    const int64_t idx = aux_id * RP + rl;
    if (aux_plan) {
      const int32_t n_own = aux_plan[mb];
      const int32_t n_left = aux_plan[mb + 1 + n_own];
      if (idx < n_left) aux_row(aux_plan[mb + 2 + n_own + idx]);
    } else if (idx <= n_multi) {
      aux_row(idx);
    }
    return;
  }
  const int64_t r_begin = r_begin0, r_end = r_end0;
  int64_t r = r_begin + rl;
  if (active) {
  if (pre) {
    store(out + r * ldo, norm(pb0, pv0));
    store(out + (r + RP) * ldo, norm(pb1, pv1));
    store(out + (r + 2 * RP) * ldo, norm(pb2, pv2));
    store(out + (r + 3 * RP) * ldo, norm(pb3, pv3));
    r += 4 * (int64_t)RP;
  }
  for (; r + 3 * (int64_t)RP < r_end; r += 4 * (int64_t)RP) {
    const int b0 = bid[r], b1 = bid[r + RP], b2 = bid[r + 2 * RP], b3 = bid[r + 3 * RP];
    const float4 v0 = *reinterpret_cast<const float4*>(x + r * ldx + c);
    const float4 v1 = *reinterpret_cast<const float4*>(x + (r + RP) * ldx + c);
    const float4 v2 = *reinterpret_cast<const float4*>(x + (r + 2 * RP) * ldx + c);
    const float4 v3 = *reinterpret_cast<const float4*>(x + (r + 3 * RP) * ldx + c);
    store(out + r * ldo, norm(b0, v0));
    store(out + (r + RP) * ldo, norm(b1, v1));
    store(out + (r + 2 * RP) * ldo, norm(b2, v2));
    store(out + (r + 3 * RP) * ldo, norm(b3, v3));
  }
  for (; r < r_end; r += RP) store(out + r * ldo, norm(bid[r], *reinterpret_cast<const float4*>(x + r * ldx + c)));
  }
// ... 747 lines not shown
```

octfusion_amd/graph_unet_hr.py:

```python
import inspect

import torch
import torch.nn as nn

from . import ops
from .modules import (GraphConv, GraphDownsample, GraphResBlockEmbed, GraphUpsample, _Linear,
                      graphnormalization, skip_window)


def level_plan(input_depth, channel_mult, num_res_blocks):
    enc, dec = [], []
    d = input_depth
    last = len(channel_mult) - 1
    for level in range(len(channel_mult)):
        enc += [('res', d, level)] * num_res_blocks[level]
        if level != last:
            enc.append(('down', d, level))
            d -= 1
    for level in range(last, -1, -1):
        for i in range(num_res_blocks[level] + 1):
            dec.append(('res', d, level))
            if level and i == num_res_blocks[level]:
                dec.append(('up', d, level))
                d += 1
# ... 142 lines not shown
        def skip_slot(i):
            c_h, c_skip, _ = self._cat_plan[i]
            return cat_bufs[i][:, c_h:]

        d = self.input_depth
        if as_middle:
            h = x
            ops.rows_copy(x, skip_slot(0), x.shape[0])
            hs = [skip_slot(0)]
        else:
            h = self.input_blocks[0](x, doctree, d, out=skip_slot(0))
            hs = [h]
        if emb_fork is not None:
            emb_main.wait_stream(emb_fork)
        for k, ((kind, dd, _), module) in enumerate(zip(self._enc, self.input_blocks[1:])):
            slot = skip_slot(k + 1)
            if kind == 'res':
                h = module(h, emb, doctree, dd, emb_act=emb_act, out=slot, emb_out=emb_outs[id(module)])
            else:
                h = module(h, doctree, dd, out=slot)
            hs.append(h)
        d = self._d_mid

        if unet_lr is not None:
            c_mid = self.middle_block1.out_channels
            mid = torch.empty(n_at[d], 2 * c_mid, dtype=torch.float32, device=dev)
            h = self.middle_block1(h, emb, doctree, d, emb_act=emb_act, out=mid[:, :c_mid], emb_out=emb_outs[id(self.middle_block1)])
            ahead_ok = ops.SKIP_AHEAD and not ops.LANE_CUS and not isinstance(unet_lr, UNet3DModel)
            ahead_main, ahead_side = ops.skip_ahead_stream(dev) if ahead_ok else (None, None)
            if ahead_side is not None:
                todo, si = [], len(hs)
                for (kind, dd, _), module in zip(self._dec, self.output_blocks):
                    if kind == 'res':
                        si -= 1
                        win = skip_window(self._cat_plan[si][0], self._cat_plan[si][1], module.block1_norm.group)
                        if win is not None:
                            todo.append((n_at[dd] * (win[1] - win[0]) * module.out_channels, si, dd, module))
                with torch.cuda.stream(ahead_side):
                    for _, si, dd, module in sorted(todo, key=lambda t_: -t_[0]):
                        module.prepare_skip(cat_bufs[si], doctree, dd, ops.SKIP_AHEAD_CUS, c_h=self._cat_plan[si][0],
                                            skip_stats=ops.get_stats(hs[si]))
            if 'out' in inspect.signature(unet_lr.forward_as_middle).parameters:
                h_lr = unet_lr.forward_as_middle(h, doctree, timesteps, label, context, out=mid[:, c_mid:])
            else:
                h_lr = unet_lr.forward_as_middle(h, doctree, timesteps, label, context)
            if h_lr.data_ptr() == mid[:, c_mid:].data_ptr() and h_lr.shape[1] == c_mid:
                h = ops.cat_channels(h, h_lr, buf=mid)
            else:
                h = ops.cat_channels(h, h_lr)
            if ahead_side is not None:
                ahead_main.wait_stream(ahead_side)
            last = len(cat_bufs) - 1
            h = self.middle_block2(h, emb, doctree, d, emb_act=emb_act, emb_out=emb_outs[id(self.middle_block2)],
                                   out=cat_bufs[last][:, :self._cat_plan[last][0]])

        n_skip = len(hs)
        j = 0
        pending = h
        for idx, ((kind, dd, _), module) in enumerate(zip(self._dec, self.output_blocks)):
            nxt_is_res = idx + 1 < len(self._dec) and self._dec[idx + 1][0] == 'res'
            out_slot = None
            if nxt_is_res:
                c_h_n = self._cat_plan[n_skip - 1 - (j + (1 if kind == 'res' else 0))][0]
                out_slot = cat_bufs[n_skip - 1 - (j + (1 if kind == 'res' else 0))][:, :c_h_n]
            if kind == 'res':
                si = n_skip - 1 - j
                c_h = self._cat_plan[si][0]
                left = cat_bufs[si][:, :c_h]
                if pending.data_ptr() != left.data_ptr():
                    ops.rows_copy(pending, left, pending.shape[0])
                    st = ops.get_stats(pending)
                    if st is not None:
                        setattr(left, ops.STATS_ATTR, st)
                    pending = left
                if module.ahead_pending(cat_bufs[si], h_stats=ops.get_stats(pending)):
                    hcat = cat_bufs[si]
                else:
                    hcat = ops.cat_channels(pending, hs[si], buf=cat_bufs[si])
                pending = module(hcat, emb, doctree, dd, emb_act=emb_act, out=out_slot, emb_out=emb_outs[id(module)])
                j += 1
            else:
                pending = module(pending, doctree, dd, out=out_slot)
        h = pending
        h = self.end_norm(h, doctree, self.input_depth, act='silu', out=out_mid if as_middle else None)
        if as_middle:
            return h
        out = self.out(h, doctree, self.input_depth)
        assert out.shape[0] == x.shape[0]
        return out
```

octfusion_amd/modules.py:

```python
import math

import torch
import torch.nn as nn

from . import ops


def _gn_groups(channels, group=32):
    if channels <= 32:
        group = channels // 4
    elif channels % group != 0:
        group = 30
    assert channels % group == 0
    return group


class GraphConv(nn.Module):

    def __init__(self, in_channels, out_channels, n_edge_type=7, avg_degree=7, n_node_type=0,
                 use_bias=False):
        super().__init__()
        assert n_edge_type == 7, 'the dual octree graph has 7 edge types'
        self.in_channels = in_channels
        self.out_channels = out_channels
        self.use_bias = use_bias
        self.n_edge_type = n_edge_type
        self.avg_degree = avg_degree
        self.n_node_type = n_node_type
        node_channel = n_node_type if n_node_type > 1 else 0
        self.weights = nn.Parameter(torch.empty(n_edge_type * (in_channels + node_channel), out_channels))
        if use_bias:
            self.bias = nn.Parameter(torch.empty(out_channels))
        self.reset_parameters()
        self._pw = ops.PackedWeight()
        self._pw2 = ops.PackedPlanes()
        self._pno = ops.PackedNarrowOut()
        self.emit_stats = True

    def planes_mode(self, doctree, d, cin=None):
        mode = ops.planes_mode()
        if not mode:
            return 0
        cin = self.in_channels if cin is None else (cin if ops.planes_pairs(mode) else 64)
        N = doctree.csr(d)[2]
        tiles = ((N + 255) // 256) * ((self.out_channels + 127) // 128)
        if (cin % (32 if ops.planes_pairs(mode) else 64) or self.out_channels % 4 or self.out_channels < 64 or
                tiles < ops.PLANES_MIN_TILES):
            return 0
        return mode

    def reset_parameters(self):
        fan_in = self.avg_degree * self.in_channels
        fan_out = self.avg_degree * self.out_channels
        a = math.sqrt(3.0) * math.sqrt(2.0 / float(fan_in + fan_out))
        nn.init.uniform_(self.weights, -a, a)
        if self.use_bias:
            nn.init.zeros_(self.bias)

    @torch.no_grad()
    def forward(self, x, doctree, d, emb=None, res=None, out=None, split_input=False):
        nt = self.n_node_type if self.n_node_type > 1 else 0
        seg_ptr, col, N, E = doctree.csr(d)
        assert x.shape[0] == N, 'x has %d rows, graph depth %d has %d nodes' % (x.shape[0], d, N)
        stats = None
        if self.emit_stats and N * self.out_channels >= (1 << 14) and self.out_channels % 4 == 0:
            stats = ops.stats_zeros(doctree.batch_size * self.out_channels * 2, x.device)
        mode = ops.planes_of(x)
        cin_k = self.in_channels
        if not mode and emb is None and res is None:
            if ops.narrow_in_ok(self.in_channels, self.out_channels, nt):
                y = ops.graphconv_narrow_in(x, seg_ptr, col, self.weights, self.in_channels, nt,
                                            doctree.node_type8(d) if nt else None, self.bias if self.use_bias else None,
                                            doctree.batch_id32(d) if stats is not None else None, out, stats,
                                            ext=doctree.ext(d), max_seg=doctree.max_seg(d))
                if stats is not None:
                    setattr(y, ops.STATS_ATTR, stats)
                return y
            if ops.NARROW_OUT and self.out_channels <= 8 and self.in_channels % 32 == 0 and N >= 4096:
                pno = self._pno.get(self.weights, self.in_channels, nt)
                bias = self.bias if self.use_bias else None
                tkey = ('narrow_tt', d, nt, self.weights.data_ptr(), self.weights._version,
                        None if bias is None else (bias.data_ptr(), bias._version))
                tt = doctree._tf.get(tkey)
                if tt is None and (nt or bias is not None):
                    tt = doctree._tf[tkey] = pno.type_term(doctree.type_frac(d, nt) if nt else None, nt, N, self.in_channels, bias)
                return ops.graphconv_narrow_out(x, seg_ptr, col, pno, self.in_channels, tt, out)
        if not mode and split_input:
            mode = self.planes_mode(doctree, d)
            if mode:
                x = ops.planes_split(x, mode)
        if not mode and self.in_channels < 32:
            mode = self.planes_mode(doctree, d, cin=32)
            if mode:
                cin_k = 32 if ops.planes_pairs(mode) else 64
                x = ops.planes_split(x, mode, Cpad=cin_k)
        if mode:
            pw2 = self._pw2.get(self.weights, self.in_channels, nt, mode, cin_pad=cin_k)
            y = ops.graphconv_planes(x, mode, seg_ptr, col, doctree.ext(d), pw2, cin_k, nt,
                                     doctree.type_frac_planes(d, nt, mode) if nt else None,
                                     self.bias if self.use_bias else None, emb,
                                     doctree.batch_id32(d) if (emb is not None or stats is not None) else None,
                                     res, out, stats=stats)
            if stats is not None:
                setattr(y, ops.STATS_ATTR, stats)
            return y
        pw = self._pw.get(self.weights, 'graphconv', self.in_channels, nt)
        tf = doctree.type_frac(d, nt) if nt else None
        y = ops.graphconv(x, doctree.nbr(d), seg_ptr, col, pw, self.in_channels, tf,
                          self.bias if self.use_bias else None, emb,
                          doctree.batch_id32(d) if (emb is not None or stats is not None) else None, res, out,
                          ext=doctree.ext(d), stats=stats)
        if stats is not None:
            setattr(y, ops.STATS_ATTR, stats)
        return y

    def extra_repr(self):
        return 'channel_in={}, channel_out={}, n_edge_type={}, avg_degree={}, n_node_type={}'.format(
            self.in_channels, self.out_channels, self.n_edge_type, self.avg_degree, self.n_node_type)


class DualOctreeGroupNorm(nn.Module):

    def __init__(self, in_channels, group=32, nempty=False):
        super().__init__()
        self.eps = 1e-5
        self.nempty = nempty
        self.in_channels = in_channels
        self.group = _gn_groups(in_channels, group)
        self.channels_per_group = in_channels // self.group
        self.weights = nn.Parameter(torch.ones(1, in_channels))
        self.bias = nn.Parameter(torch.zeros(1, in_channels))

    @torch.no_grad()
    def forward(self, data, doctree, depth, act=None, out=None, planes=0):
        assert doctree.batch_id32(depth).shape[0] == data.shape[0]
        stats = ops.get_stats(data)
        if ops.planes_pairs(planes) and out is not None and not ops.planes_ok(out, planes):
            out = None
        aux_graph = None
        if planes:
            seg_ptr, col, _, _ = doctree.csr(depth)
            _, multi_seg, n_multi = doctree.ext(depth)
            oct_plan = doctree.oct_plan(depth) if ops.AUX_PLAN == 'oct' else None
            block_plan = doctree.aux_plan(depth) if ops.AUX_PLAN and oct_plan is None else None
            aux_graph = ops.AuxGraph(seg_ptr, col, multi_seg, n_multi, oct_plan, block_plan)
        y = ops.group_norm(data, doctree.batch_id32(depth), doctree.count(depth), doctree.batch_size,
                           self.weights, self.bias, self.group, self.eps, act, out, stats=stats, planes=planes,
                           aux_graph=aux_graph)
        if out is data and stats is not None:
            delattr(data, ops.STATS_ATTR)
        return y

    def extra_repr(self):
        return 'in_channels={}, group={}, nempty={}'.format(self.in_channels, self.group, self.nempty)


class _Linear(nn.Module):

    def __init__(self, cin, cout, bias=True):
        super().__init__()
        self.in_features, self.out_features = cin, cout
        self.weight = nn.Parameter(torch.empty(cout, cin))
        self.bias = nn.Parameter(torch.empty(cout)) if bias else None
        nn.init.kaiming_uniform_(self.weight, a=math.sqrt(5))
        if bias:
            bound = 1 / math.sqrt(cin)
            nn.init.uniform_(self.bias, -bound, bound)
        self._pw = ops.PackedWeight()

# ... 389 lines not shown
```

octfusion_amd/ops.py:

```python
import contextlib
import os
from typing import NamedTuple

import torch

from . import _lib
from ._lib import call, call_may_decline, ptr, stream

ACT = {None: 0, 'none': 0, 'silu': 1, 'gelu': 2}

GRAPHCONV_PROFILE = None
_NO_BRACKET = contextlib.nullcontext()


@contextlib.contextmanager
def _timed_layer(prof, *rec):
    e0 = torch.cuda.Event(enable_timing=True)
    e1 = torch.cuda.Event(enable_timing=True)
    e0.record()
    yield
    e1.record()
    prof.append((e0, e1) + rec)


# ... 368 lines not shown


def workspace(device, nbytes=96 << 20):
    def make():
        _no_capture('the split-K / hand-off workspace')
        return torch.empty(nbytes, dtype=torch.uint8, device=device)
    t = _scratch('ws', device, True, make)
    if t.numel() < nbytes:
        t = _SCRATCH[_scratch_key('ws', device, True)] = make()
    return t


def scan_i32(x):
    _chk(x, torch.int32)
    n = x.numel()
    out = torch.empty(n + 1, dtype=torch.int32, device=x.device)
    ws = torch.empty(_lib.lib().ofx_scan_ws_bytes(n), dtype=torch.uint8, device=x.device)
    call('ofx_scan_i32', ptr(x), ptr(out), n, ptr(ws), stream())
    return out


class PackedWeight:

    def __init__(self):
        self.t = None
        self.key = None
        self.K = self.N = self.Kp = 0

    def get(self, w, mode, cin=0, nt=0):
        key = (w.data_ptr(), w._version, tuple(w.shape), mode, cin, nt, _lib.lib().ofx_get_precision() == 3)
        if key == self.key:
            return self
        _chk(w)
        w = w.detach()
        if not w.is_contiguous():
            w = w.contiguous()
        L = _lib.lib()
        if mode == 'kn' or mode == 'graphconv':
            K, N = w.shape
            sk, sn = N, 1
        elif mode == 'nk':
            N, K = w.shape
            sk, sn = 1, K
        else:
            raise ValueError(mode)
        if mode == 'graphconv':
            Kp = L.ofx_graphconv_packed_k(cin, nt)
        else:
            cin = nt = 0
            Kp = L.ofx_packed_k(K)
        out = torch.empty(L.ofx_packed_floats(Kp, N), dtype=torch.float32, device=w.device)
        call('ofx_pack_weights', ptr(w), sk, sn, K, N, cin, nt, ptr(out), Kp, stream())
        self.t, self.key, self.K, self.N, self.Kp = out, key, K, N, Kp
        return self


def gemm(a, pw, bias=None, res=None, out=None, a_rows=None, out_rows=None, m=None, out_planes=0):
    a, lda = _row_major(a)
    M = m if m is not None else (a_rows.numel() if a_rows is not None else a.shape[0])
    if a.shape[1] != pw.K:
        raise ValueError('K mismatch: %d vs %d' % (a.shape[1], pw.K))
    out, ldc = _out2d(out, M, pw.N, a.device)
    res, ldr = _row_major(res)
    _chk(bias)
    _chk(a_rows, torch.int32)
    _chk(out_rows, torch.int32)
    ws = workspace(a.device)
    _meta('dense_gemm', 2.0 * M * pw.K * pw.N, 4.0 * (M * pw.K + pw.K * pw.N + M * pw.N * (2 if res is not None else 1)),
          (M, pw.K, pw.N))
    if out_planes:
        args = ('ofx_gemm_f32_planes', ptr(a), lda, ptr(a_rows), M, pw.K, ptr(pw.t), pw.Kp, pw.N, ptr(bias),
                ptr(res), ldr, ptr(out), ldc, ptr(out_rows), ptr(ws), ws.numel(), out_planes, stream())
    else:
        args = ('ofx_gemm_f32', ptr(a), lda, ptr(a_rows), M, pw.K, ptr(pw.t), pw.Kp, pw.N, ptr(bias),
                ptr(res), ldr, ptr(out), ldc, ptr(out_rows), ptr(ws), ws.numel(), stream())
    if pw.N <= 64 or pw.K <= 64:
        with policy_scope('small_gemm'):
            call(*args)
    else:
        call(*args)
    return out


def gather_gemm(x, tab, ntap, pw, n_out, bias=None, res=None, out=None, out_rows=None, out_planes=0):
    x, ldx = _row_major(x)
    cin = x.shape[1]
    assert pw.K == ntap * cin and cin % 32 == 0
    _chk(tab, torch.int32)
    out, ldc = _out2d(out, n_out, pw.N, x.device)
    res, ldr = _row_major(res)
    _chk(bias)
    _chk(out_rows, torch.int32)
    ws = workspace(x.device)
    _meta('dense_gemm', 2.0 * n_out * pw.K * pw.N, 4.0 * (n_out * pw.K + pw.K * pw.N + n_out * pw.N), (n_out, pw.K, pw.N))
    call('ofx_gather_gemm_f32', ptr(x), ldx, cin, ntap, x.shape[0], n_out, ptr(tab), ptr(zero_row(x.device)), ptr(pw.t), pw.Kp,
         pw.N, ptr(bias), ptr(res), ldr, ptr(out), ldc, ptr(out_rows), ptr(ws), ws.numel(), out_planes, stream())
    return out


GEMM_PLANES = os.environ.get('OFX_GEMM_PLANES', '0') == '1'


class PackedGemmPlanes:

    def __init__(self):
        self.t = None
        self.key = None

    def get(self, w2d, mode):
        key = (w2d.data_ptr(), w2d._version, tuple(w2d.shape), tuple(w2d.stride()), mode)
        if key != self.key:
            _chk(w2d)
            K, N = w2d.shape
            nb = _lib.lib().ofx_gemm_planes_packed_bytes(K, N, mode)
            assert nb > 0
            t = torch.empty(nb, dtype=torch.uint8, device=w2d.device)
            assert t.data_ptr() % 128 == 0
            call('ofx_pack_gemm_planes', ptr(w2d.detach()), w2d.stride(0), w2d.stride(1), K, N, mode, ptr(t), stream())
            self.t, self.key, self.K, self.N = t, key, K, N
        return self


def gemm_planes(a_planes, pgp, out, out_planes=0, bias=None):
    mode = planes_of(a_planes)
    M, K = a_planes.shape
    assert planes_pairs(mode) and K == pgp.K and a_planes.stride(1) == 1
    dev = a_planes.device
    out, ldc = _out2d(out, M, pgp.N, dev)
    tabs = _scratch('row_tab', dev, False, dict)
    tab = tabs.get(M)
    if tab is None:
        if len(tabs) > 64:
            tabs.clear()
        _no_capture('the row table of a dense planes GEMM')
        tab = torch.zeros(M * 7 + 4, dtype=torch.int32, device=dev)
        tab[:M * 7].view(M, 7)[:, 0] = torch.arange(M, dtype=torch.int32, device=dev)
        tabs[M] = tab
    ws = workspace(dev)
    sync = sync_words(dev)
    _meta('dense_gemm', 2.0 * M * K * pgp.N, 4.0 * (M * K + K * pgp.N + M * pgp.N), (M, K, pgp.N, 'planes'))
    return call_may_decline('ofx_gemm_planes', ptr(a_planes), a_planes.stride(0) * 4, M, M, K, ptr(tab), ptr(pgp.t), pgp.N,
                            ptr(bias), ptr(out), ldc, out_planes, ptr(ws), ws.numel(), ptr(sync), sync.numel() * 4, mode,
                            stream())


LINEAR_SMALL = True


def linear_small(a, weight, bias=None, res=None, act_in=None, act_out=None, out=None):
    a, lda = _row_major(a)
    w, ldw = _row_major(weight.detach())
    M, K = a.shape
    N = w.shape[0]
    assert w.shape[1] == K and M <= 16
    out, ldo = _out2d(out, M, N, a.device)
    res, ldr = _row_major(res)
    _chk(bias)
    _meta('small_linear', 2.0 * M * K * N, 4.0 * (N * K + M * K + M * N), (M, K, N))
    call('ofx_linear_small', ptr(a), lda, M, K, ptr(w), ldw, N, ptr(bias.detach() if bias is not None else None), ptr(res),
         ldr, ACT[act_in], ACT[act_out], ptr(out), ldo, stream())
    return out


def learned_sinusoid(t, w):
    _chk(t), _chk(w)
    t, w = t.contiguous(), w.detach().contiguous()
# ... 51 lines not shown

NARROW_IN = os.environ.get('OFX_NARROW_IN', '1') == '1'
NARROW_OUT = os.environ.get('OFX_NARROW_OUT', '1') == '1'


def narrow_in_ok(cin, cout, nt):
    return NARROW_IN and cin <= 8 and cout in (64, 128) and 7 * (cin + nt) <= 96


NARROW_IN_TAB = os.environ.get('OFX_NARROW_IN_TAB', '1') == '1'
NARROW_IN_TAB_MIN_ROWS = int(os.environ.get('OFX_NARROW_IN_TAB_MIN_ROWS', str(1 << 19)))


NARROW_IN_TAB_MAX_SEG = 255


def graphconv_narrow_in(x, seg_ptr, col, weights, cin, nt, node_type=None, bias=None, batch_id=None, out=None, stats=None,
                        ext=None, max_seg=None):
    x, ldx = _row_major(x)
    w = weights.detach()
    if not w.is_contiguous():
        w = w.contiguous()
    _chk(w)
    N, cout = x.shape[0], w.shape[1]
    assert x.shape[1] == cin and w.shape[0] == 7 * (cin + nt)
    out, ldc = _out2d(out, N, cout, x.device)
    if nt:
        _chk(node_type, torch.uint8)
    _chk(bias)
    _chk(stats, torch.float64)
    if stats is not None:
        _chk(batch_id, torch.int32)
    E = col.numel()
    flops = 2.0 * N * w.shape[0] * cout
    nbytes = 4.0 * (E * cin + N * cout + w.numel()) + 8.0 * E
    with _layer_bracket(flops, nbytes, cout, ('graph', N, cin, cout)):
        ws = workspace(x.device)
        _meta('graphconv_narrow', flops, nbytes, (N, cin, cout, 'narrow_in'))
        if (ext is not None and NARROW_IN_TAB and N >= NARROW_IN_TAB_MIN_ROWS and max_seg is not None and
                (max_seg <= NARROW_IN_TAB_MAX_SEG or not nt)):
            nbr_ext, multi_seg, n_multi = ext
            aux = torch.empty((N + n_multi + 1) * (8 if cin <= 4 else 16), dtype=torch.float32, device=x.device)
            call('ofx_graphconv_narrow_in_tab', ptr(x), ldx, cin, N, ptr(seg_ptr), ptr(col), ptr(nbr_ext), ptr(multi_seg),
                 n_multi, ptr(aux), ptr(node_type) if nt else None, nt, ptr(w), cout, ptr(bias),
                 ptr(batch_id) if stats is not None else None, ptr(out), ldc, ptr(stats), cout, ptr(ws), ws.numel(),
                 stream())
        else:
            call('ofx_graphconv_narrow_in', ptr(x), ldx, cin, N, ptr(seg_ptr), ptr(col), ptr(node_type) if nt else None, nt,
                 ptr(w), cout, ptr(bias), ptr(batch_id) if stats is not None else None, ptr(out), ldc, ptr(stats), cout,
                 ptr(ws), ws.numel(), stream())
    return out


class PackedNarrowOut:

    def __init__(self):
        self.key = None
        self.pw = PackedWeight()

    def get(self, w, C, nt):
        key = (w.data_ptr(), w._version, tuple(w.shape), C, nt)
        if key != self.key:
            wd = w.detach()
            if not wd.is_contiguous():
                wd = wd.contiguous()
            _chk(wd)
            cout = wd.shape[1]
            self.width = 32 if 7 * cout <= 32 else 64
            self.wd = torch.empty(C, self.width, dtype=torch.float32, device=w.device)
            call('ofx_narrow_out_pack', ptr(wd), C, nt, cout, self.width, ptr(self.wd), stream())
            self.w = wd
            self.key = key
        return self

    def type_term(self, type_frac, nt, N, C, bias):
        cout = self.w.shape[1]
        tt = torch.empty(N, cout, dtype=torch.float32, device=self.w.device)
        _chk(bias)
        call('ofx_narrow_out_type_term', ptr(type_frac) if nt else None, type_frac.stride(0) if nt else 0, nt, N, ptr(self.w),
             C, cout, ptr(bias), ptr(tt), stream())
        return tt


def graphconv_narrow_out(x, seg_ptr, col, pno, C, type_term=None, out=None):
    N = x.shape[0]
    cout = pno.w.shape[1]
    E = col.numel()
    flops = 2.0 * N * pno.w.shape[0] * cout
    pwid = pno.width
    agg_bytes = 4.0 * (N * pwid + E + 7 * N + 2 * N * cout)
    nbytes = agg_bytes + 4.0 * (N * C + N * pwid + pno.w.numel())
    with _layer_bracket(flops, nbytes, cout, ('graph', N, C, cout)):
        P = gemm(x, pno.pw.get(pno.wd, 'kn'))
        out, ldc = _out2d(out, N, cout, x.device)
        _chk(type_term)
        assert type_term is None or (type_term.is_contiguous() and tuple(type_term.shape) == (N, cout))
        _meta('graphconv_narrow', flops, agg_bytes, (N, C, cout, 'narrow_out'))
        call('ofx_graphconv_narrow_out', ptr(P), P.stride(0), cout, N, ptr(seg_ptr), ptr(col), ptr(type_term), ptr(out),
             ldc, stream())
    return out


def gemm_tn(p, q):
    _chk(p), _chk(q)
    assert p.shape[0] == q.shape[0]
    K0, N0 = p.shape[1], q.shape[1]

    def pad4(t):
        c = t.shape[1]
        if c % 4 == 0 and t.stride(0) % 4 == 0 and t.stride(1) == 1 and t.data_ptr() % 16 == 0:
            return t
        out = torch.zeros(t.shape[0], (c + 3) // 4 * 4, dtype=torch.float32, device=t.device)
        out[:, :c] = t
        return out
    p, q = pad4(p), pad4(q)
    if (K0, N0) != (p.shape[1], q.shape[1]):
        return gemm_tn(p, q)[:K0, :N0].contiguous()
    p, ldp = _row_major(p)
    q, ldq = _row_major(q)
    K, N = p.shape[1], q.shape[1]
    out = torch.empty(K, N, dtype=torch.float32, device=p.device)
    ws = workspace(p.device)
    call('ofx_gemm_tn_f32', ptr(p), ldp, ptr(q), ldq, p.shape[0], K, N, ptr(out), ptr(ws), ws.numel(), stream())
    return out


GRAD_TOP_EXP = 8


def grad_pow2(dy):
    lo, hi = torch.aminmax(dy) if dy.numel() else (dy.new_zeros(()), dy.new_zeros(()))
    _, e = torch.frexp(torch.maximum(-lo, hi))
    s = (GRAD_TOP_EXP - e).clamp(-100, 100)
    return torch.ldexp(dy, s), torch.ldexp(torch.ones_like(hi), -s)


def gemm_grad(dy, pw):
    dys, inv = grad_pow2(dy)
    return gemm(dys, pw).mul_(inv)


def linear_backward(x, dy, weight, need_dx=True):
    dW = gemm_tn(dy, x)
    dx = gemm_grad(dy, PackedWeight().get(weight, 'kn')) if need_dx else None
    return dx, dW, dy.sum(0)


def graphconv_backward(x, dy, doctree, d, weights, n_node_type, need_dx=True, need_dw=True):
    x, ldx = _row_major(x)
    dy, ldy = _row_major(dy)
    _chk(x), _chk(dy), _chk(weights)
    N, cin = x.shape
    cout = dy.shape[1]
    nt = n_node_type if n_node_type > 1 else 0
    assert weights.shape == (7 * (cin + nt), cout)
    seg_ptr, col, Ng, E = doctree.csr(d)
    assert N == Ng and dy.shape[0] == N
    ws = workspace(x.device)
    dx = dW = None
    if need_dx:
        rv = doctree.rev(d)
        wt = weights.detach().view(7, cin + nt, cout)[:, :cin, :].permute(0, 2, 1).reshape(7 * cout, cin).contiguous()
        pwt = PackedWeight().get(wt, 'graphconv', cout, 0)
        dx = torch.empty(N, cin, dtype=torch.float32, device=x.device)
        dys, inv = grad_pow2(dy)
        lds = dys.stride(0)
        fast = cout % 32 == 0 and lds % 4 == 0
        aux = torch.empty((rv['V'] + 1) * lds, dtype=torch.float32, device=x.device) if fast else None
        call('ofx_graphconv_bwd_data', ptr(dys), lds, cout, N, ptr(rv['nbr']), ptr(rv['rev_ptr']), ptr(rv['rev_row']),
             ptr(rv['rev_w']), ptr(rv['nbr_ext']) if fast else None, ptr(rv['multi_seg']) if fast else None,
             rv['V'] if fast else 0, ptr(aux), ptr(pwt.t), pwt.Kp, cin, ptr(dx), cin, ptr(ws), ws.numel(), stream())
        dx.mul_(inv)
    if need_dw:
        L = _lib.lib()
        Kp = L.ofx_graphconv_packed_k(cin, nt)
        Kf = Kp - (((7 * nt + 31) // 32) * 32 if nt else 0)
# ... 417 lines not shown
```

Baseline: 121.8.

## Fuse head GroupNorm+SiLU into narrow-out GEMM operand load

Adds a GEMM variant that applies group-norm normalisation and optional SiLU to A tiles as they are loaded into LDS. Per-batch mean/rstd slots and gamma/beta are staged in shared memory. The final UNet head uses it, via graphconv_narrow_out, to skip a separate norm+act pass and the write and re-read of the normalised activation. In exchange it adds a gn_finalize launch, extra LDS use, per-element ALU work in the load path, and a global fallback when a tile spans more than four batches.

```diff
diff --git a/include/ofx.h b/include/ofx.h
--- a/include/ofx.h
+++ b/include/ofx.h
@@ -178,6 +178,12 @@
                         const float* Wp, int64_t Kp, int64_t N, const float* bias,
                         const float* res, int64_t ldr, float* out, int64_t ldc,
                         const int32_t* out_rows, void* ws, size_t ws_bytes, int out_mode, void* stream);
+int ofx_gemm_f32_gn(const float* A, int64_t lda, const int32_t* a_rows, int64_t M, int64_t K,
+                    const float* Wp, int64_t Kp, int64_t N, const float* bias,
+                    const float* res, int64_t ldr, float* out, int64_t ldc,
+                    const int32_t* out_rows, const int32_t* batch_id, int batch_size, const float* mean,
+                    const float* rstd, int stats_ld, const float* gamma, const float* beta, int act, void* ws,
+                    size_t ws_bytes, void* stream);
 
 int ofx_graphconv_fwd(const float* x, int64_t ldx, int cin, int64_t n_nodes,
                       const int32_t* nbr, const int32_t* seg_ptr, const int32_t* col,
@@ -280,6 +286,11 @@
                         const float* zero_row, const float* Wp, int64_t Kp, int cout, const float* bias,
                         const float* res, int64_t ldr, float* out, int64_t ldc, const int32_t* out_rows, void* ws,
                         size_t ws_bytes, int out_mode, void* stream);
+int ofx_gather_gemm_f32_gn(const float* x, int64_t ldx, int cin, int ntap, int64_t n_src, int64_t n_out,
+                           const int32_t* tab, const float* zero_row, const float* Wp, int64_t Kp, int cout,
+                           const float* bias, const float* res, int64_t ldr, float* out, int64_t ldc,
+                           const int32_t* out_rows, const int32_t* batch_id, const float* gamma, const float* beta,
+                           void* ws, size_t ws_bytes, int out_mode, void* stream);
 int ofx_set_attention_split(int on);
 int ofx_attention(const float* qkv, int64_t ldq, int batch_size, int T, int heads, int ch,
                   float* out, int64_t ldo, void* stream);
diff --git a/octfusion_amd/_lib.py b/octfusion_amd/_lib.py
--- a/octfusion_amd/_lib.py
+++ b/octfusion_amd/_lib.py
@@ -109,6 +109,10 @@
     'ofx_graphconv_packed_k': (c_l, [c_i, c_i], False),
     'ofx_pack_weights': (c_i, [c_p, c_l, c_l, c_l, c_l, c_i, c_i, c_p, c_l, c_p], True),
     'ofx_gemm_f32': (c_i, [c_p, c_l, c_p, c_l, c_l, c_p, c_l, c_l, c_p, c_p, c_l, c_p, c_l, c_p, c_p, c_sz, c_p], True),
+    'ofx_gemm_f32_gn': (c_i, [c_p, c_l, c_p, c_l, c_l, c_p, c_l, c_l, c_p, c_p, c_l, c_p, c_l, c_p, c_p, c_i, c_p, c_p, c_i,
+                              c_p, c_p, c_i, c_p, c_sz, c_p], True),
+    'ofx_gather_gemm_f32_gn': (c_i, [c_p, c_l, c_i, c_i, c_l, c_l, c_p, c_p, c_p, c_l, c_i, c_p, c_p, c_l, c_p, c_l, c_p,
+                                     c_p, c_p, c_p, c_p, c_sz, c_i, c_p], True),
     'ofx_gemm_f32_planes': (c_i, [c_p, c_l, c_p, c_l, c_l, c_p, c_l, c_l, c_p, c_p, c_l, c_p, c_l, c_p, c_p, c_sz, c_i, c_p], True),
     'ofx_graphconv_fwd': (c_i, [c_p, c_l, c_i, c_l, c_p, c_p, c_p, c_p, c_p, c_l, c_p, c_p, c_l, c_i, c_p, c_l,
                                 c_i, c_p, c_p, c_l, c_p, c_p, c_l, c_p, c_l, c_p, c_l, c_p, c_sz, c_p], True),
diff --git a/octfusion_amd/csrc/ofx_gemm.hip b/octfusion_amd/csrc/ofx_gemm.hip
--- a/octfusion_amd/csrc/ofx_gemm.hip
+++ b/octfusion_amd/csrc/ofx_gemm.hip
@@ -1,4 +1,7 @@
+#include <type_traits>
+
 #include "ofx_gemm_common.h"
+#include "ofx_gn_common.h"
 
 constexpr int BM = 128;
 constexpr int BK = 32;
@@ -370,8 +373,11 @@
     return __builtin_amdgcn_mfma_f32_32x32x16_f16(__builtin_bit_cast(f16x8h_t, a), __builtin_bit_cast(f16x8h_t, b), c, 0, 0, 0);
 }
 
-template <int MODE, int WM, int WN, int MI, int NI, int H16>
-__global__ void __launch_bounds__(256, 2) gemm_pairs_x3_kernel(const GemmArgs g) {
+constexpr int GN_SLOTS = 4;
+template <int MODE, int WM, int WN, int MI, int NI, int H16, class ARGS = GemmArgs>
+__global__ void __launch_bounds__(256, 2) gemm_pairs_x3_kernel(const ARGS g) {
+  constexpr bool GN = !std::is_same<ARGS, GemmArgs>::value;
+  static_assert(!GN || MODE == MODE_DENSE, "normalisation on load: dense mode only");
   constexpr int BN = WN * NI * 32;
   constexpr int A_BYTES = BM * 80;
   constexpr int BUF_BYTES = 2 * A_BYTES;
@@ -430,6 +436,54 @@
   if (MODE == MODE_DENSE && g.a_rows) { dr0 = g.a_rows[m_0]; dr1 = g.a_rows[m_1]; dr2 = g.a_rows[m_2]; dr3 = g.a_rows[m_3]; }
   const gfp dp0 = xp + dr0 * ldx, dp1 = xp + dr1 * ldx, dp2 = xp + dr2 * ldx, dp3 = xp + dr3 * ldx;
   const int kclamp = (int)g.K - 4;
+
+  float* const gn_t = reinterpret_cast<float*>(smem8 + 2 * BUF_BYTES);
+  const int gnK = (int)g.K;
+  const GnLoadArgs gn_none = {};
+  const GnLoadArgs& gn = [&]() -> const GnLoadArgs& {
+    if constexpr (GN) return g.gn;
+    else return gn_none;
+  }();
+  int gn_so0 = -1, gn_so1 = -1, gn_so2 = -1, gn_so3 = -1;
+  int gn_b0 = 0, gn_b1 = 0, gn_b2 = 0, gn_b3 = 0;
+  auto gn_prologue = [&]() {
+    const int64_t rl = m0 + BM - 1 < mmax ? m0 + BM - 1 : mmax;
+    const int bf = gn.bid[g.a_rows ? (int64_t)g.a_rows[m0] : m0];
+    const int bl = gn.bid[g.a_rows ? (int64_t)g.a_rows[rl] : rl];
+    gn_b0 = gn.bid[dr0]; gn_b1 = gn.bid[dr1]; gn_b2 = gn.bid[dr2]; gn_b3 = gn.bid[dr3];
+    int nslot = bl - bf + 1;
+    nslot = nslot < 1 ? 1 : (nslot > GN_SLOTS ? GN_SLOTS : nslot);
+    if (bf + nslot > gn.batch) nslot = gn.batch - bf;
+    for (int c = threadIdx.x; c < gnK; c += 256) {
+      gn_t[c] = gn.w[c];
+      gn_t[gnK + c] = gn.b[c];
+    }
+    for (int t = threadIdx.x; t < nslot * gnK; t += 256) {
+      const int s = t / gnK, c = t - s * gnK;
+      gn_t[(2 + 2 * s) * gnK + c] = gn.mean[(int64_t)(bf + s) * gn.ld + c];
+      gn_t[(3 + 2 * s) * gnK + c] = gn.rstd[(int64_t)(bf + s) * gn.ld + c];
+    }
+    auto slot_off = [&](int b) { return (b >= bf && b - bf < nslot) ? (2 + 2 * (b - bf)) * gnK : -1; };
+    gn_so0 = slot_off(gn_b0); gn_so1 = slot_off(gn_b1); gn_so2 = slot_off(gn_b2); gn_so3 = slot_off(gn_b3);
+    __syncthreads();
+  };
+  auto gn_apply4 = [&](float4& v, int so, int b, int it) {
+    const int itc = it < nkt_g ? it : nkt_g - 1;
+    int cc = itc * BK + c4 * 4;
+    cc = cc < kclamp ? cc : kclamp;
+    const float4 ww = *reinterpret_cast<const float4*>(gn_t + cc);
+    const float4 bb = *reinterpret_cast<const float4*>(gn_t + gnK + cc);
+    float4 m, rs;
+    if (so >= 0) {
+      m = *reinterpret_cast<const float4*>(gn_t + so + cc);
+      rs = *reinterpret_cast<const float4*>(gn_t + so + gnK + cc);
+    } else {
+      m = *reinterpret_cast<const float4*>(gn.mean + (int64_t)b * gn.ld + cc);
+      rs = *reinterpret_cast<const float4*>(gn.rstd + (int64_t)b * gn.ld + cc);
+    }
+    if (gn.act == OFX_ACT_SILU) v = ofx_gn_norm_act4(v, m, rs, ww, bb, OFX_ACT_SILU);
+    else v = ofx_gn_norm_act4(v, m, rs, ww, bb, OFX_ACT_NONE);
+  };
 
   int64_t bcol[NI];
 #pragma unroll
@@ -529,9 +583,19 @@
 #pragma unroll
       for (int j = 0; j < NI; ++j) { F.h[c][j] = wk[bcol[j]]; F.l[c][j] = wk[lo_off + bcol[j]]; }
     };
-    auto store_half = [&](int buf, const float4& v0, const float4& v1, int row_off) {
+    auto store_half = [&](int buf, const float4& v0, const float4& v1, int row_off, int it_) {
       char* a = a_st + buf * BUF_BYTES + row_off * 80;
       uint2 hi, lo;
+      if constexpr (GN != 0) {
+        float4 n0 = v0, n1 = v1;
+        gn_apply4(n0, row_off ? gn_so2 : gn_so0, row_off ? gn_b2 : gn_b0, it_);
+        gn_apply4(n1, row_off ? gn_so3 : gn_so1, row_off ? gn_b3 : gn_b1, it_);
+        split16x4<H16>(n0, hi, lo);
+        *reinterpret_cast<uint2*>(a) = hi; *reinterpret_cast<uint2*>(a + A_BYTES) = lo;
+        split16x4<H16>(n1, hi, lo);
+        *reinterpret_cast<uint2*>(a + 32 * 80) = hi; *reinterpret_cast<uint2*>(a + 32 * 80 + A_BYTES) = lo;
+        return;
+      }
       split16x4<H16>(v0, hi, lo);
       *reinterpret_cast<uint2*>(a) = hi; *reinterpret_cast<uint2*>(a + A_BYTES) = lo;
       split16x4<H16>(v1, hi, lo);
@@ -570,11 +634,11 @@
       OFX_FENCE();
       OFX_MFMA_GROUP(al, h, 1);
       OFX_FENCE();
-      store_half(buf ^ 1, Rold.a0, Rold.a1, 0);
+      store_half(buf ^ 1, Rold.a0, Rold.a1, 0, it + 1);
       OFX_FENCE();
       OFX_MFMA_GROUP(ah, l, 1);
       OFX_FENCE();
-      store_half(buf ^ 1, Rold.a2, Rold.a3, 64);
+      store_half(buf ^ 1, Rold.a2, Rold.a3, 64, it + 1);
       OFX_FENCE();
       OFX_MFMA_GROUP(ah, h, 1);
 #undef OFX_MFMA_GROUP
@@ -592,8 +656,9 @@
     OFX_FENCE();
     load_rows(g_begin + 1, I1, R1);
     OFX_FENCE();
-    store_half(0, R0.a0, R0.a1, 0);
-    store_half(0, R0.a2, R0.a3, 64);
+    if constexpr (GN != 0) gn_prologue();
+    store_half(0, R0.a0, R0.a1, 0, g_begin);
+    store_half(0, R0.a2, R0.a3, 64, g_begin);
     __syncthreads();
     int it = g_begin;
     for (; it + 1 < g_end; it += 2) {
@@ -757,13 +822,30 @@
   KERNEL<<<g.ntm * g.ntn * g.nsplit, 256, LDS, st>>>(g);
   return OFX_OK;
 }
+template <void (*KERNEL)(const GemmGnArgs)>
+static int launch_tiled_gn(GemmArgs& g, const GnLoadArgs& gn, hipStream_t st) {
+  const size_t lds = 2 * (2 * BM * 80) + (size_t)(2 + 2 * GN_SLOTS) * g.K * sizeof(float);
+  if (lds > 64 * 1024) return OFX_EINVAL;
+  GemmGnArgs a;
+  static_cast<GemmArgs&>(a) = g;
+  a.gn = gn;
+  KERNEL<<<g.ntm * g.ntn * g.nsplit, 256, lds, st>>>(a);
+  return OFX_OK;
+}
 template <int MODE, int WM, int WN, int MI, int NI>
-static int launch_cfg(GemmArgs& g, int flavour, hipStream_t st) {
+static int launch_cfg(GemmArgs& g, int flavour, hipStream_t st, const GnLoadArgs* gn) {
   constexpr size_t lds_f32 = (2 * BM * A_LD + 2 * 8 * (WN * NI * 32) * 4) * sizeof(float);
   constexpr size_t lds_16 = 2 * (2 * BM * 80);
+  if (gn) {
+    if constexpr (MODE == MODE_DENSE) {
+      if (flavour == 3) return launch_tiled_gn<gemm_pairs_x3_kernel<MODE, WM, WN, MI, NI, 1, GemmGnArgs>>(g, *gn, st);
+      if (flavour == 2) return launch_tiled_gn<gemm_pairs_x3_kernel<MODE, WM, WN, MI, NI, 0, GemmGnArgs>>(g, *gn, st);
+    }
+    return OFX_EINVAL;
+  }
   switch (flavour) {
-    case 3: return launch_tiled<gemm_pairs_x3_kernel<MODE, WM, WN, MI, NI, 1>, lds_16>(g, st);
-    case 2: return launch_tiled<gemm_pairs_x3_kernel<MODE, WM, WN, MI, NI, 0>, lds_16>(g, st);
+    case 3: return launch_tiled<gemm_pairs_x3_kernel<MODE, WM, WN, MI, NI, 1, GemmArgs>, lds_16>(g, st);
+    case 2: return launch_tiled<gemm_pairs_x3_kernel<MODE, WM, WN, MI, NI, 0, GemmArgs>, lds_16>(g, st);
     case 1: return launch_tiled<gemm_fast_kernel<MODE, WM, WN, MI, NI>, lds_f32>(g, st);
   }
   if constexpr (MODE == MODE_DENSE) return launch_tiled<gemm_dense_generic_kernel<WM, WN, MI, NI>, lds_f32>(g, st);
@@ -833,9 +915,10 @@
 }
 
 template <int MODE>
-static int launch_gemm(GemmArgs& g, float* ws, size_t ws_bytes, hipStream_t st) {
+static int launch_gemm(GemmArgs& g, float* ws, size_t ws_bytes, hipStream_t st, const GnLoadArgs* gn = nullptr) {
   if (g.M <= 0 || g.N <= 0) return OFX_OK;
   if (MODE == MODE_GATHER && !(g.fast && g.nbr_ext && g.aux && (!g.out_rows || g.gather_out_rows))) return OFX_EINVAL;
+  if (MODE == MODE_GATHER && gn) return OFX_EINVAL;
   {
     auto al16 = [](const void* p) { return (reinterpret_cast<uintptr_t>(p) & 15) == 0; };
     g.vec4 = g.N % 4 == 0 && al16(g.out) && g.ldc % 4 == 0 && (!g.res || (al16(g.res) && g.ldr % 4 == 0)) &&
@@ -873,9 +956,9 @@
   g.oscale_p = (fast && g.W16) ? g.Wp + 2 * g.Kp * g.N : nullptr;
   const int flavour = !fast ? 0 : (!g.W16 ? 1 : (g_precision == 3 ? 3 : 2));
   int rc;
-  if (bn == 32) rc = launch_cfg<MODE, 4, 1, 1, 1>(g, flavour, st);
-  else if (bn == 64) rc = launch_cfg<MODE, 2, 2, 2, 1>(g, flavour, st);
-  else rc = launch_cfg<MODE, 2, 2, 2, 2>(g, flavour, st);
+  if (bn == 32) rc = launch_cfg<MODE, 4, 1, 1, 1>(g, flavour, st, gn);
+  else if (bn == 64) rc = launch_cfg<MODE, 2, 2, 2, 1>(g, flavour, st, gn);
+  else rc = launch_cfg<MODE, 2, 2, 2, 2>(g, flavour, st, gn);
   if (rc) return rc;
   if (nsplit > 1) {
     const bool ws16 = (((uintptr_t)g.ws) & 15) == 0;
@@ -988,6 +1071,26 @@
   g.M = M; g.K = K; g.Wp = Wp; g.Kp = Kp; g.N = N; g.bias = bias;
   g.res = res; g.ldr = ldr; g.out = out; g.ldc = ldc; g.out_rows = out_rows; g.out_planes = out_mode;
   return launch_gemm<MODE_DENSE>(g, (float*)ws, ws_bytes, ofx_stream(stream));
+}
+extern "C" int ofx_gemm_f32_gn(const float* A, int64_t lda, const int32_t* a_rows, int64_t M, int64_t K, const float* Wp,
+                               int64_t Kp, int64_t N, const float* bias, const float* res, int64_t ldr, float* out,
+                               int64_t ldc, const int32_t* out_rows, const int32_t* batch_id, int batch_size,
+                               const float* mean, const float* rstd, int stats_ld, const float* gamma, const float* beta,
+                               int act, void* ws, size_t ws_bytes, void* stream) {
+  if (M == 0 && K >= 1 && N >= 1) return OFX_OK;
+  if (M < 0 || K < 4 || (K & 3) || N < 1 || !Wp || !out || !A || Kp != pad32(K) || lda < K || (lda & 3) || ldc < N ||
+      (res && ldr < N) || ((uintptr_t)Wp & 15) || ((uintptr_t)A & 15))
+    return OFX_EINVAL;
+  if (!batch_id || batch_size < 1 || !gamma || !beta || (act != OFX_ACT_NONE && act != OFX_ACT_SILU)) return OFX_EINVAL;
+  if (stats_ld == 0) stats_ld = (int)K;
+  if (stats_ld < K || (stats_ld & 3) || !mean || !rstd || (((uintptr_t)mean | (uintptr_t)rstd) & 15)) return OFX_EINVAL;
+  if (g_precision == 1) return OFX_EINVAL;
+  GemmArgs g = {};
+  g.A = A; g.lda = lda; g.a_rows = a_rows;
+  g.M = M; g.K = K; g.Wp = Wp; g.Kp = Kp; g.N = N; g.bias = bias;
+  g.res = res; g.ldr = ldr; g.out = out; g.ldc = ldc; g.out_rows = out_rows;
+  const GnLoadArgs gn = {gamma, beta, batch_id, mean, rstd, stats_ld, batch_size, act};
+  return launch_gemm<MODE_DENSE>(g, (float*)ws, ws_bytes, ofx_stream(stream), &gn);
 }
 extern "C" int ofx_gemm_f32(const float* A, int64_t lda, const int32_t* a_rows, int64_t M, int64_t K, const float* Wp,
                             int64_t Kp, int64_t N, const float* bias, const float* res, int64_t ldr, float* out,
@@ -1512,6 +1615,22 @@
   return launch_gemm<MODE_GATHER>(g, (float*)ws, ws_bytes, ofx_stream(stream));
 }
 
+extern "C" int ofx_gather_gemm_f32_gn(const float* x, int64_t ldx, int cin, int ntap, int64_t n_src, int64_t n_out,
+                                      const int32_t* tab, const float* zero_row, const float* Wp, int64_t Kp, int cout,
+                                      const float* bias, const float* res, int64_t ldr, float* out, int64_t ldc,
+                                      const int32_t* out_rows, const int32_t* batch_id, const float* gamma,
+                                      const float* beta, void* ws, size_t ws_bytes, int out_mode, void* stream) {
+  if (batch_id || gamma || beta) {
+    GemmArgs g = {};
+    g.M = n_out; g.N = cout; g.fast = 1; g.nbr_ext = tab; g.aux = zero_row;
+    const GnLoadArgs gn = {gamma, beta, batch_id};
+    const int rc = launch_gemm<MODE_GATHER>(g, nullptr, 0, ofx_stream(stream), &gn);
+    return rc ? rc : OFX_EINVAL;
+  }
+  return ofx_gather_gemm_f32(x, ldx, cin, ntap, n_src, n_out, tab, zero_row, Wp, Kp, cout, bias, res, ldr, out, ldc,
+                             out_rows, ws, ws_bytes, out_mode, stream);
+}
+
 __global__ void __launch_bounds__(256) gather_mean_kernel(const float* __restrict__ x, int64_t ldx, int cin, int64_t nseg,
                                                           const int32_t* __restrict__ seg_ptr,
                                                           const int32_t* __restrict__ col, float* __restrict__ out) {
diff --git a/octfusion_amd/csrc/ofx_gemm_common.h b/octfusion_amd/csrc/ofx_gemm_common.h
--- a/octfusion_amd/csrc/ofx_gemm_common.h
+++ b/octfusion_amd/csrc/ofx_gemm_common.h
@@ -29,6 +29,13 @@
   float* stats_part; size_t stats_part_bytes;
 };
 
+struct GnLoadArgs {
+  const float* w; const float* b; const int32_t* bid;
+  const float* mean; const float* rstd; int ld;
+  int batch, act;
+};
+struct GemmGnArgs : GemmArgs { GnLoadArgs gn; };
+
 static __global__ void __launch_bounds__(256) weight_absmax_kernel(const float* __restrict__ W, int64_t sk, int64_t sn, int64_t K,
                                                             int64_t N, unsigned* __restrict__ acc) {
   __shared__ float red[256];
diff --git a/octfusion_amd/csrc/ofx_gn_common.h b/octfusion_amd/csrc/ofx_gn_common.h
--- /dev/null
+++ b/octfusion_amd/csrc/ofx_gn_common.h
@@ -0,0 +1,34 @@
+#pragma once
+#include "ofx_common.h"
+
+__device__ __forceinline__ float ofx_apply_act(float v, int act) {
+  if (act == OFX_ACT_SILU) return v / (1.f + __expf(-v));
+  if (act == OFX_ACT_GELU) return 0.5f * v * (1.f + erff(v * 0.70710678118654752440f));
+  return v;
+}
+
+__device__ __forceinline__ float ofx_gn_norm_act(float v, float mean, float rstd, float w, float b, int act) {
+  return ofx_apply_act((v - mean) * rstd * w + b, act);
+}
+__device__ __forceinline__ float4 ofx_gn_norm_act4(const float4& v, const float4& m, const float4& rs, const float4& ww,
+                                                   const float4& bb, int act) {
+  return make_float4(ofx_gn_norm_act(v.x, m.x, rs.x, ww.x, bb.x, act), ofx_gn_norm_act(v.y, m.y, rs.y, ww.y, bb.y, act),
+                     ofx_gn_norm_act(v.z, m.z, rs.z, ww.z, bb.z, act), ofx_gn_norm_act(v.w, m.w, rs.w, ww.w, bb.w, act));
+}
+
+struct GnFin { const double* sums; const float* count; int G; float eps, count_eps; int ld; };
+__device__ __forceinline__ void gn_group_stats(const GnFin& f, int b, int g, int C, float& mean, float& rstd) {
+  const int cpg = C / f.G;
+  double S = 0, SS = 0;
+  for (int c = g * cpg; c < (g + 1) * cpg; ++c) {
+    S += f.sums[((int64_t)b * f.ld + c) * 2];
+    SS += f.sums[((int64_t)b * f.ld + c) * 2 + 1];
+  }
+  const float cnt = f.count[b] * (float)cpg;
+  const float inv = 1.0f / (cnt + f.count_eps);
+  const double m = S * (double)inv;
+  const double ssd = SS - 2.0 * m * S + (double)cnt * m * m;
+  const double var = (ssd > 0 ? ssd : 0) * (double)inv;
+  mean = (float)m;
+  rstd = (float)(1.0 / sqrt(var + (double)f.eps));
+}
diff --git a/octfusion_amd/csrc/ofx_norm.hip b/octfusion_amd/csrc/ofx_norm.hip
--- a/octfusion_amd/csrc/ofx_norm.hip
+++ b/octfusion_amd/csrc/ofx_norm.hip
@@ -1,4 +1,5 @@
 #include "ofx_planes.h"
+#include "ofx_gn_common.h"
 
 constexpr int GN_ROWS_PER_BLOCK = 64;
 
@@ -155,29 +156,7 @@
   return OFX_OK;
 }
 
-__device__ __forceinline__ float ofx_apply_act(float v, int act) {
-  if (act == OFX_ACT_SILU) return v / (1.f + __expf(-v));
-  if (act == OFX_ACT_GELU) return 0.5f * v * (1.f + erff(v * 0.70710678118654752440f));
-  return v;
-}
-
 constexpr int GN_APPLY_ROWS = 64;
-struct GnFin { const double* sums; const float* count; int G; float eps, count_eps; int ld; };
-__device__ __forceinline__ void gn_group_stats(const GnFin& f, int b, int g, int C, float& mean, float& rstd) {
-  const int cpg = C / f.G;
-  double S = 0, SS = 0;
-  for (int c = g * cpg; c < (g + 1) * cpg; ++c) {
-    S += f.sums[((int64_t)b * f.ld + c) * 2];
-    SS += f.sums[((int64_t)b * f.ld + c) * 2 + 1];
-  }
-  const float cnt = f.count[b] * (float)cpg;
-  const float inv = 1.0f / (cnt + f.count_eps);
-  const double m = S * (double)inv;
-  const double ssd = SS - 2.0 * m * S + (double)cnt * m * m;
-  const double var = (ssd > 0 ? ssd : 0) * (double)inv;
-  mean = (float)m;
-  rstd = (float)(1.0 / sqrt(var + (double)f.eps));
-}
 template <int MODE, bool FIN>
 __global__ void __launch_bounds__(256) gn_apply_kernel(const float* __restrict__ x, int64_t ldx, int64_t n, int C,
                                                        const int32_t* __restrict__ bid, const float* __restrict__ mean,
@@ -283,10 +262,7 @@
         rs = *reinterpret_cast<const float4*>(rstd + (int64_t)b * fin.ld + c);
       }
     }
-    return make_float4(ofx_apply_act((v.x - m.x) * rs.x * ww.x + bb.x, act),
-                       ofx_apply_act((v.y - m.y) * rs.y * ww.y + bb.y, act),
-                       ofx_apply_act((v.z - m.z) * rs.z * ww.z + bb.z, act),
-                       ofx_apply_act((v.w - m.w) * rs.w * ww.w + bb.w, act));
+    return ofx_gn_norm_act4(v, m, rs, ww, bb, act);
   };
   auto store = [&](char* orow, const float4& y) {
     if (MODE == 0) {
diff --git a/octfusion_amd/graph_unet_hr.py b/octfusion_amd/graph_unet_hr.py
--- a/octfusion_amd/graph_unet_hr.py
+++ b/octfusion_amd/graph_unet_hr.py
@@ -248,6 +248,11 @@
             else:
                 pending = module(pending, doctree, dd, out=out_slot)
         h = pending
+        if not as_middle and ops.HEAD_GN_ON_LOAD:
+            out = self.out.forward_normed(h, self.end_norm, doctree, self.input_depth, act='silu')
+            if out is not None:
+                assert out.shape[0] == x.shape[0]
+                return out
         h = self.end_norm(h, doctree, self.input_depth, act='silu', out=out_mid if as_middle else None)
         if as_middle:
             return h
diff --git a/octfusion_amd/modules.py b/octfusion_amd/modules.py
--- a/octfusion_amd/modules.py
+++ b/octfusion_amd/modules.py
@@ -56,6 +56,34 @@
         nn.init.uniform_(self.weights, -a, a)
         if self.use_bias:
             nn.init.zeros_(self.bias)
+
+    def narrow_out_ok(self, x, N):
+        return (not ops.planes_of(x) and ops.NARROW_OUT and self.out_channels <= 8 and self.in_channels % 32 == 0
+                and N >= 4096 and not ops.narrow_in_ok(self.in_channels, self.out_channels,
+                                                       self.n_node_type if self.n_node_type > 1 else 0))
+
+    @torch.no_grad()
+    def forward_normed(self, x, norm, doctree, d, act=None, out=None):
+        N = doctree.csr(d)[2]
+        stats = ops.get_stats(x)
+        if (stats is None or x.shape[0] != N or not self.narrow_out_ok(x, N) or not ops.gemm_gn_ok(x, self.in_channels)
+                or norm.in_channels != self.in_channels or act not in (None, 'silu')):
+            return None
+        gn = ops.GnOnLoad(doctree.batch_id32(d), doctree.count(d), doctree.batch_size, stats, norm.weights, norm.bias,
+                          norm.group, norm.eps, act)
+        return self._narrow_out(x, doctree, d, out, gn)
+
+    def _narrow_out(self, x, doctree, d, out, gn=None):
+        nt = self.n_node_type if self.n_node_type > 1 else 0
+        seg_ptr, col, N, E = doctree.csr(d)
+        pno = self._pno.get(self.weights, self.in_channels, nt)
+        bias = self.bias if self.use_bias else None
+        tkey = ('narrow_tt', d, nt, self.weights.data_ptr(), self.weights._version,
+                None if bias is None else (bias.data_ptr(), bias._version))
+        tt = doctree._tf.get(tkey)
+        if tt is None and (nt or bias is not None):
+            tt = doctree._tf[tkey] = pno.type_term(doctree.type_frac(d, nt) if nt else None, nt, N, self.in_channels, bias)
+        return ops.graphconv_narrow_out(x, seg_ptr, col, pno, self.in_channels, tt, out, gn=gn)
 
     @torch.no_grad()
     def forward(self, x, doctree, d, emb=None, res=None, out=None, split_input=False):
@@ -77,14 +105,7 @@
                     setattr(y, ops.STATS_ATTR, stats)
                 return y
             if ops.NARROW_OUT and self.out_channels <= 8 and self.in_channels % 32 == 0 and N >= 4096:
-                pno = self._pno.get(self.weights, self.in_channels, nt)
-                bias = self.bias if self.use_bias else None
-                tkey = ('narrow_tt', d, nt, self.weights.data_ptr(), self.weights._version,
-                        None if bias is None else (bias.data_ptr(), bias._version))
-                tt = doctree._tf.get(tkey)
-                if tt is None and (nt or bias is not None):
-                    tt = doctree._tf[tkey] = pno.type_term(doctree.type_frac(d, nt) if nt else None, nt, N, self.in_channels, bias)
-                return ops.graphconv_narrow_out(x, seg_ptr, col, pno, self.in_channels, tt, out)
+                return self._narrow_out(x, doctree, d, out)
         if not mode and split_input:
             mode = self.planes_mode(doctree, d)
             if mode:
diff --git a/octfusion_amd/ops.py b/octfusion_amd/ops.py
--- a/octfusion_amd/ops.py
+++ b/octfusion_amd/ops.py
@@ -474,6 +474,63 @@
     return out
 
 
+HEAD_GN_ON_LOAD = os.environ.get('OFX_HEAD_GN_ON_LOAD', '1') == '1'
+GEMM_GN_KMAX = 576
+
+
+class GnOnLoad(NamedTuple):
+    batch_id: torch.Tensor
+    count: torch.Tensor
+    batch_size: int
+    sums: torch.Tensor
+    weight: torch.Tensor
+    bias: torch.Tensor
+    groups: int
+    eps: float
+    act: str = None
+
+
+def gemm_gn_ok(a, pw_K):
+    return (a.dim() == 2 and a.stride(1) == 1 and a.stride(0) % 4 == 0 and a.data_ptr() % 16 == 0 and pw_K % 4 == 0
+            and pw_K <= GEMM_GN_KMAX and a.shape[1] == pw_K and get_precision() != 'fp32'
+            and POLICY['small_gemm'] is None)
+
+
+def gemm_gn(a, pw, gn, bias=None, res=None, out=None, a_rows=None, out_rows=None):
+    a, lda = _row_major(a)
+    M = a_rows.numel() if a_rows is not None else a.shape[0]
+    K = pw.K
+    if a.shape[1] != K:
+        raise ValueError('K mismatch: %d vs %d' % (a.shape[1], K))
+    out, ldc = _out2d(out, M, pw.N, a.device)
+    res, ldr = _row_major(res)
+    _chk(bias)
+    _chk(a_rows, torch.int32)
+    _chk(out_rows, torch.int32)
+    _chk(gn.batch_id, torch.int32)
+    _chk(gn.sums, torch.float64)
+    assert gn.sums.numel() == gn.batch_size * K * 2
+    w = gn.weight.detach().reshape(-1)
+    b = gn.bias.detach().reshape(-1)
+    mean = torch.empty(gn.batch_size * K, dtype=torch.float32, device=a.device)
+    rstd = torch.empty(gn.batch_size * K, dtype=torch.float32, device=a.device)
+    _meta('gn_finalize', 0, 24.0 * gn.batch_size * K, (gn.batch_size, K))
+    call('ofx_gn_finalize', ptr(gn.sums), ptr(gn.count), gn.batch_size, K, gn.groups, gn.eps, gn.eps, ptr(mean), ptr(rstd),
+         stream())
+    ws = workspace(a.device)
+    _meta('dense_gemm', 2.0 * M * K * pw.N, 4.0 * (M * K + K * pw.N + M * pw.N * (2 if res is not None else 1)),
+          (M, K, pw.N, 'gn_on_load'))
+    args = ('ofx_gemm_f32_gn', ptr(a), lda, ptr(a_rows), M, K, ptr(pw.t), pw.Kp, pw.N, ptr(bias), ptr(res), ldr, ptr(out),
+            ldc, ptr(out_rows), ptr(gn.batch_id), gn.batch_size, ptr(mean), ptr(rstd), K, ptr(w), ptr(b), ACT[gn.act],
+            ptr(ws), ws.numel(), stream())
+    if pw.N <= 64 or K <= 64:
+        with policy_scope('small_gemm'):
+            call(*args)
+    else:
+        call(*args)
+    return out
+
+
 def gather_gemm(x, tab, ntap, pw, n_out, bias=None, res=None, out=None, out_rows=None, out_planes=0):
     x, ldx = _row_major(x)
     cin = x.shape[1]
@@ -691,7 +748,7 @@
         return tt
 
 
-def graphconv_narrow_out(x, seg_ptr, col, pno, C, type_term=None, out=None):
+def graphconv_narrow_out(x, seg_ptr, col, pno, C, type_term=None, out=None, gn=None):
     N = x.shape[0]
     cout = pno.w.shape[1]
     E = col.numel()
@@ -700,7 +757,7 @@
     agg_bytes = 4.0 * (N * pwid + E + 7 * N + 2 * N * cout)
     nbytes = agg_bytes + 4.0 * (N * C + N * pwid + pno.w.numel())
     with _layer_bracket(flops, nbytes, cout, ('graph', N, C, cout)):
-        P = gemm(x, pno.pw.get(pno.wd, 'kn'))
+        P = gemm(x, pno.pw.get(pno.wd, 'kn')) if gn is None else gemm_gn(x, pno.pw.get(pno.wd, 'kn'), gn)
         out, ldc = _out2d(out, N, cout, x.device)
         _chk(type_term)
         assert type_term is None or (type_term.is_contiguous() and tuple(type_term.shape) == (N, cout))
```

Result: no change. 122.0 (median of 6 runs) (+0.2%).
